# huawei-noah/xingtian

Hardware: NVIDIA H100
Metric: learner env-steps/sec (Atari 84x84x4 PPO) (higher is better)
Workload: dtype f32 (bf16x3 split on wgmma, fp32 accumulate in registers)

## Files before the change

### include/xtb200.h

```cpp
#ifndef XTB200_H_
#define XTB200_H_

#include <stddef.h>
#include <stdint.h>

#ifdef __cplusplus
extern "C" {
#endif

#define XTB_VERSION 101

enum xtb_status {
  XTB_OK = 0,
  XTB_ERR_ARG = -1,
  XTB_ERR_CUDA = -2,
  XTB_ERR_STATE = -3,
  XTB_ERR_NOMEM = -4
};

enum xtb_layer_kind { XTB_CONV = 0, XTB_DENSE = 1, XTB_DUELING = 2, XTB_LOGSTD = 3 };
enum xtb_act {
  XTB_ACT_NONE = 0, XTB_ACT_RELU = 1, XTB_ACT_TANH = 2, XTB_ACT_SIGMOID = 3, XTB_ACT_SOFTSIGN = 4, XTB_ACT_SOFTPLUS = 5,
  XTB_ACT_LEAKY_RELU = 6, XTB_ACT_ELU = 7, XTB_ACT_SELU = 8, XTB_ACT_SWISH = 9, XTB_ACT_GELU = 10
};
// ... 120 lines not shown
  const void* obs;
  const void* action;
  const float* old_logp;
  const float* adv;
  const float* old_v;
  const float* target_v;
} xtb_ppo_rollout;
int xtb_ppo_train(xtb_net* net, xtb_adam* opt, const xtb_ppo_rollout* ro, int n_sample, int batch_size, int n_epoch,
                  const int32_t* perm, const xtb_ppo_hyper* hp, int pi_tensor, int v_tensor, int logstd_tensor,
                  float* loss_per_step, int use_graph, void* stream);

int xtb_impala_train(xtb_net* net, xtb_adam* opt, const void* obs, const int32_t* gather_idx, const float* bp_logits,
                     const int32_t* action, const uint8_t* done, const float* reward, int n_sample, int step_len,
                     float gamma, int logit_tensor, int base_tensor, float* loss_out, int use_graph, void* stream);
int xtb_dqn_train(xtb_net* net, xtb_net* target, xtb_adam* opt, const void* obs, const void* next_obs,
                  const int32_t* idx, const int32_t* action, const float* reward, const uint8_t* done,
                  const float* disc, int n_sample, float gamma, float huber_delta, int q_tensor, float* qn_t,
                  float* qn_o, float* loss_out, int use_graph, void* stream);

int xtb_impala_keras_fit(xtb_net* net, xtb_adam* opt, const void* obs, const int32_t* order, const float* action_mat,
                         const float* adv, const float* target_v, int n, int fit_batch, int logit_tensor, int v_tensor,
                         float ent_coef, float* loss_out, int use_graph, void* stream);
typedef struct xtb_impala_traj {
  const void* obs;
  const float* behav_prob;
  const float* action_mat;
  const float* reward;
  const uint8_t* done;
} xtb_impala_traj;
int xtb_impala_keras_train(xtb_net* net, xtb_adam* opt, const xtb_impala_traj* tr, int n_traj, int ep_len, int slice,
                           int fit_batch, const int32_t* order, int32_t* obs_idx, float gamma, float ent_coef,
                           int logit_tensor, int v_tensor, float* pg_adv, float* target_v, float* loss_per_slice,
                           int use_graph, void* stream);

int xtb_ppo_rollout_infer(xtb_net* net, const void* obs, const int32_t* step_idx, int n_env, int n_step, int pi_tensor,
                          int v_tensor, int logstd_tensor, uint64_t seed, unsigned long long* offset_dev, void* action,
                          float* logp, float* value, int use_graph, void* stream);

int xtb_ppo_predict_host(xtb_net* net, const void* obs_host, size_t obs_bytes, void* obs_dev, int n_env, int pi_tensor,
                         int v_tensor, int logstd_tensor, uint64_t seed, unsigned long long* offset_dev, float* out_dev,
                         float* out_host, float* head_host, int use_graph, void* stream);

int xtb_diag_gaussian_sample(const float* mean, const float* log_std, int batch, int adim, const float* normals,
                             uint64_t seed, uint64_t offset, float* action, float* logp, void* stream);
int xtb_ppo_gauss_loss_grad(const float* mean, const float* v, const float* log_std, const int32_t* gather_idx,
                            const float* action, const float* old_logp, const float* adv, const float* old_v,
                            const float* target_v, int batch, int adim, const xtb_ppo_hyper* hp, float inv_count,
                            float* dmean, float* dv, float* dlog_std, float* loss_out, void* stream);

typedef struct xtb_muzero xtb_muzero;
typedef struct xtb_muzero_desc {
  int32_t unroll;
  int32_t rep_h;
  int32_t dyn_h, dyn_r;
  int32_t pred_p, pred_v;
  float value_min, value_max;
  float reward_min, reward_max;
} xtb_muzero_desc;
int xtb_muzero_create(xtb_net* rep, xtb_net* dyn, xtb_net* pred, const xtb_muzero_desc* desc, int max_batch, xtb_muzero** out);
void xtb_muzero_destroy(xtb_muzero* mz);
typedef struct xtb_muzero_batch {
  const void* obs;
  const int32_t* action;
  const float* target_value;
  const float* target_reward;
  const float* target_policy;
  int32_t unroll;
} xtb_muzero_batch;
int xtb_muzero_train(xtb_muzero* mz, xtb_adam* opt, const xtb_muzero_batch* batch_in, int batch, float loss_offset,
                     float* loss_out, float* value_out, int use_graph, void* stream);
int xtb_muzero_initial_inference(xtb_muzero* mz, const void* obs, int batch, float* hidden_out, float* value_out,
                                 float* policy_out, int use_graph, void* stream);
int xtb_muzero_recurrent_inference(xtb_muzero* mz, const float* hidden, const int32_t* action, int batch, float* hidden_out,
                                   float* reward_out, float* value_out, float* policy_out, int use_graph, void* stream);
typedef struct xtb_muzero_tree xtb_muzero_tree;
int xtb_muzero_tree_create(const xtb_muzero* mz, int max_envs, int max_simulations, xtb_muzero_tree** out);
void xtb_muzero_tree_destroy(xtb_muzero_tree* tree);
int xtb_muzero_search(xtb_muzero* mz, xtb_muzero_tree* tree, const void* obs, int n_envs, int num_simulations,
                      const double* noise, double pb_c_base, double pb_c_init, double discount, double exploration_frac,
                      int32_t* visit_counts_out, double* root_value_out, int use_graph, void* stream);
typedef struct xtb_qmix xtb_qmix;
typedef struct xtb_qmix_desc {
  int32_t batch;
  int32_t episode_limit;
  int32_t n_agents;
  int32_t use_double_q;
  float gamma;
  long long gru_off;
} xtb_qmix_desc;
int xtb_qmix_create(xtb_net* fc1, xtb_net* fc2, xtb_net* hyper, const xtb_qmix_desc* desc, xtb_qmix** out);
void xtb_qmix_destroy(xtb_qmix* q);
typedef struct xtb_qmix_batch {
  const float* obs;
  const int32_t* seq_len;
  const float* avail;
  const int32_t* actions;
  const float* state;
  const float* next_state;
  const float* reward;
  const float* terminated;
  const float* mask;
} xtb_qmix_batch;
int xtb_qmix_train(xtb_qmix* q, xtb_adam* opt, const float* target, const xtb_qmix_batch* batch, float* loss_out, int use_graph,
                   void* stream);
int xtb_qmix_infer(xtb_qmix* q, const float* explore, const float* obs, float* hidden, float* q_out, int use_graph, void* stream);

typedef struct xtb_scc xtb_scc;
#define XTB_SCC_MAX_GROUPS 8
typedef struct xtb_scc_desc {
  int32_t batch;
  int32_t episode_limit;
  int32_t n_agents;
  int32_t n_groups;
  int32_t group[XTB_SCC_MAX_GROUPS];
  int32_t channel_merge;
  int32_t mc_sample_times;
  float gamma;
  long long gru_off;
  long long head_off;
} xtb_scc_desc;
int xtb_scc_create(xtb_net* fc1, xtb_net* fc2, xtb_net* const* critic, const xtb_scc_desc* desc, xtb_scc** out);
void xtb_scc_destroy(xtb_scc* q);
typedef struct xtb_scc_batch {
  const float* obs;
  const float* raw_obs;
  const int32_t* seq_len;
  const int32_t* actions;
  const float* reward;
  const float* terminated;
  const float* mask;
  const uint32_t* subsets;
} xtb_scc_batch;
int xtb_scc_train(xtb_scc* q, xtb_adam* critic_opt, xtb_adam* actor_opt, const float* target, const xtb_scc_batch* batch,
                  float* loss_out, int use_graph, void* stream);
int xtb_scc_infer(xtb_scc* q, const float* explore, const float* obs, float* hidden, float* q_out, int use_graph, void* stream);
int xtb_scc_critic(xtb_scc* q, const float* states, int rows, float* v_out, int use_graph, void* stream);

int xtb_net_backward_input(xtb_net* net, const void* obs, const int32_t* gather_idx, int batch,
                           const int32_t* head_tensors, int n_heads, float* dobs, void* stream);

typedef struct xtb_comm xtb_comm;
int xtb_comm_unique_id(const char* nccl_path, void* id128);
int xtb_comm_create(const char* nccl_path, const void* id128, int rank, int world, xtb_comm** out);
void xtb_comm_destroy(xtb_comm* comm);
int xtb_comm_world(const xtb_comm* comm);
int xtb_set_grad_comm(xtb_comm* comm);
int xtb_comm_allreduce(xtb_comm* comm, float* buf, long long count, void* stream);

int xtb_net_bench_layer(xtb_net* net, int layer, int which, const void* obs, const int32_t* gather_idx,
                        int batch, void* stream);

int xtb_set_tc_mode(int mode);
int xtb_set_fuse_heads(int on);
int xtb_get_tc_mode(void);
int xtb_tc_gemm_test(int mode, const float* a, const float* b, float* c, int M, int N, int K, int ksplit,
                     void* stream);

void* xtb_pinned_alloc(size_t bytes);
void xtb_pinned_free(void* p);
int xtb_copy_h2d(void* dst_dev, const void* src_host, size_t bytes, void* stream);
int xtb_copy_h2d_staged(void* dst_dev, const void* src_host, size_t bytes, void* stream);
int xtb_copy_d2h(void* dst_host, const void* src_dev, size_t bytes, void* stream);
int xtb_stream_sync(void* stream);

#ifdef __cplusplus
}
#endif
#endif
```

### xingtian_b200/capi.py

```python
import ctypes as C
import os

HERE = os.path.dirname(os.path.abspath(__file__))
LIB_PATH = os.environ.get("XTB_LIB_PATH") or os.path.join(HERE, "lib", "libxtb200.so")

XTB_MAX_LAYERS = 16
CONV, DENSE, DUELING, LOGSTD = 0, 1, 2, 3
ACT = {None: 0, "linear": 0, "relu": 1, "tanh": 2, "sigmoid": 3, "softsign": 4, "softplus": 5, "leaky_relu": 6, "elu": 7,
       "selu": 8, "swish": 9, "gelu": 10}
CLIP_NONE, CLIP_GLOBAL_NORM, CLIP_PER_TENSOR = 0, 1, 2


class LayerDesc(C.Structure):
    _fields_ = [("kind", C.c_int32), ("src", C.c_int32), ("act", C.c_int32), ("k", C.c_int32),
                ("stride", C.c_int32), ("cout", C.c_int32), ("pad_same", C.c_int32)]


class NetDesc(C.Structure):
    _fields_ = [("input_u8", C.c_int32), ("scale", C.c_float), ("in_h", C.c_int32), ("in_w", C.c_int32),
                ("in_c", C.c_int32), ("n_layers", C.c_int32), ("layers", LayerDesc * XTB_MAX_LAYERS)]


class LayerPlan(C.Structure):
    _fields_ = [("kind", C.c_int32), ("tc", C.c_int32), ("s2d", C.c_int32), ("w_res", C.c_int32), ("n_fwd", C.c_int32),
                ("n_dg", C.c_int32), ("R", C.c_int32), ("fwd_stages", C.c_int32), ("dg_stages", C.c_int32),
                ("dg_empty_units", C.c_int32), ("k_slices", C.c_int32)]


class PpoHyper(C.Structure):
    _fields_ = [("clip_ratio", C.c_float), ("ent_coef", C.c_float), ("vf_clip", C.c_float),
                ("critic_coef", C.c_float)]


class PpoRollout(C.Structure):
    _fields_ = [("obs", C.c_void_p), ("action", C.c_void_p), ("old_logp", C.c_void_p), ("adv", C.c_void_p),
                ("old_v", C.c_void_p), ("target_v", C.c_void_p)]


class ImpalaTraj(C.Structure):
    _fields_ = [("obs", C.c_void_p), ("behav_prob", C.c_void_p), ("action_mat", C.c_void_p), ("reward", C.c_void_p),
                ("done", C.c_void_p)]


class MuzeroDesc(C.Structure):
    _fields_ = [("unroll", C.c_int32), ("rep_h", C.c_int32), ("dyn_h", C.c_int32), ("dyn_r", C.c_int32), ("pred_p", C.c_int32),
                ("pred_v", C.c_int32), ("value_min", C.c_float), ("value_max", C.c_float), ("reward_min", C.c_float),
                ("reward_max", C.c_float)]


class MuzeroBatch(C.Structure):
    _fields_ = [("obs", C.c_void_p), ("action", C.c_void_p), ("target_value", C.c_void_p), ("target_reward", C.c_void_p),
                ("target_policy", C.c_void_p), ("unroll", C.c_int32)]


class QmixDesc(C.Structure):
    _fields_ = [("batch", C.c_int32), ("episode_limit", C.c_int32), ("n_agents", C.c_int32), ("use_double_q", C.c_int32),
                ("gamma", C.c_float), ("gru_off", C.c_longlong)]


class QmixBatch(C.Structure):
    _fields_ = [("obs", C.c_void_p), ("seq_len", C.c_void_p), ("avail", C.c_void_p), ("actions", C.c_void_p), ("state", C.c_void_p),
                ("next_state", C.c_void_p), ("reward", C.c_void_p), ("terminated", C.c_void_p), ("mask", C.c_void_p)]


class SccDesc(C.Structure):
    _fields_ = [("batch", C.c_int32), ("episode_limit", C.c_int32), ("n_agents", C.c_int32), ("n_groups", C.c_int32),
                ("group", C.c_int32 * 8), ("channel_merge", C.c_int32), ("mc_sample_times", C.c_int32), ("gamma", C.c_float),
                ("gru_off", C.c_longlong), ("head_off", C.c_longlong)]


class SccBatch(C.Structure):
    _fields_ = [("obs", C.c_void_p), ("raw_obs", C.c_void_p), ("seq_len", C.c_void_p), ("actions", C.c_void_p), ("reward", C.c_void_p),
                ("terminated", C.c_void_p), ("mask", C.c_void_p), ("subsets", C.c_void_p)]


_P = C.c_void_p
_SIGS = {
    "xtb_version": (C.c_int, []),
    "xtb_last_error": (C.c_char_p, []),
    "xtb_launch_count": (C.c_longlong, []),
    "xtb_graph_replay_count": (C.c_longlong, []),
    "xtb_net_create": (C.c_int, [C.POINTER(NetDesc), C.c_int, C.POINTER(_P)]),
    "xtb_net_destroy": (None, [_P]),
    "xtb_net_param_count": (C.c_longlong, [_P]),
    "xtb_net_layer_params": (C.c_int, [_P, C.c_int, C.POINTER(C.c_longlong), C.POINTER(C.c_longlong),
                                       C.POINTER(C.c_int), C.POINTER(C.c_int)]),
    "xtb_net_layer_plan": (C.c_int, [_P, C.c_int, C.POINTER(LayerPlan)]),
    "xtb_net_tensor_size": (C.c_int, [_P, C.c_int]),
    "xtb_net_workspace_bytes": (C.c_size_t, [_P]),
    "xtb_net_bind": (C.c_int, [_P, _P, _P, _P, C.c_size_t]),
    "xtb_net_bind_stream": (C.c_int, [_P, _P, _P, _P, C.c_size_t, _P]),
    "xtb_net_sync_weights": (C.c_int, [_P, _P]),
    "xtb_net_tensor": (_P, [_P, C.c_int]),
    "xtb_net_tensor_grad": (_P, [_P, C.c_int]),
    "xtb_net_forward": (C.c_int, [_P, _P, _P, _P, C.c_int, _P]),
    "xtb_net_backward": (C.c_int, [_P, _P, _P, C.c_int, C.POINTER(C.c_int32), C.c_int, _P]),
    "xtb_categorical_sample": (C.c_int, [_P, C.c_int, C.c_int, _P, C.c_uint64, C.c_uint64, _P, _P, _P]),
    "xtb_argmax": (C.c_int, [_P, C.c_int, C.c_int, _P, _P]),
    "xtb_gae": (C.c_int, [_P, _P, _P, C.c_int, C.c_int, C.c_float, C.c_float, C.c_int, _P, _P, _P, _P]),
    "xtb_ppo_loss_grad": (C.c_int, [_P, _P, _P, _P, _P, _P, _P, _P, C.c_int, C.c_int, C.POINTER(PpoHyper),
                                    C.c_float, _P, _P, _P, _P]),
    "xtb_vtrace_loss_grad": (C.c_int, [_P, _P, _P, _P, _P, _P, C.c_int, C.c_int, C.c_int, C.c_float,
                                       _P, _P, _P, _P, _P, _P]),
    "xtb_dqn_loss_grad": (C.c_int, [_P, _P, _P, _P, _P, _P, C.c_int, C.c_int, C.c_float, C.c_float,
                                    _P, _P, _P, _P]),
    "xtb_dqn_td_loss_grad": (C.c_int, [_P, _P, _P, _P, _P, _P, _P, _P, C.c_int, C.c_int, C.c_float, C.c_float, C.c_float,
                                      _P, _P, _P, _P]),
    "xtb_nstep_returns": (C.c_int, [_P, _P, C.c_int, C.c_int, C.c_int, C.c_float, _P, _P, _P, _P, _P]),
    "xtb_impala_train": (C.c_int, [_P, _P, _P, _P, _P, _P, _P, _P, C.c_int, C.c_int, C.c_float, C.c_int, C.c_int, _P, C.c_int, _P]),
    "xtb_dqn_train": (C.c_int, [_P, _P, _P, _P, _P, _P, _P, _P, _P, _P, C.c_int, C.c_float, C.c_float, C.c_int, _P, _P, _P,
                               C.c_int, _P]),
    "xtb_mse_loss_grad": (C.c_int, [_P, _P, C.c_int, C.c_int, C.c_float, _P, _P, _P]),
    "xtb_softmax": (C.c_int, [_P, C.c_int, C.c_int, _P, _P]),
    "xtb_impala_keras_loss_grad": (C.c_int, [_P, _P, _P, _P, _P, _P, C.c_int, C.c_int, C.c_float, C.c_float, C.c_float,
                                             _P, _P, _P, _P]),
    "xtb_impala_keras_fit": (C.c_int, [_P, _P, _P, _P, _P, _P, _P, C.c_int, C.c_int, C.c_int, C.c_int, C.c_float, _P,
                                       C.c_int, _P]),
    "xtb_impala_keras_train": (C.c_int, [_P, _P, C.POINTER(ImpalaTraj), C.c_int, C.c_int, C.c_int, C.c_int, _P, _P,
                                         C.c_float, C.c_float, C.c_int, C.c_int, _P, _P, _P, C.c_int, _P]),
    "xtb_adam_create": (C.c_int, [C.c_longlong, C.c_float, C.c_float, C.c_float, C.c_float, C.c_int,
                                  C.c_float, C.POINTER(C.c_longlong), C.c_int, _P, _P, C.POINTER(_P)]),
    "xtb_adam_destroy": (None, [_P]),
    "xtb_adam_step": (C.c_int, [_P, _P, _P, C.c_float, _P]),
    "xtb_adam_step_net": (C.c_int, [_P, _P, C.c_float, _P]),
    "xtb_adam_grad_norm": (_P, [_P]),
    "xtb_adam_set_lr": (C.c_int, [_P, C.c_float]),
    "xtb_adam_set_decay": (C.c_int, [_P, C.c_float]),
    "xtb_opt_use_rmsprop": (C.c_int, [_P, _P, C.c_float, C.c_float]),
    "xtb_opt_use_rmsprop_plain": (C.c_int, [_P, C.c_float, C.c_float]),
    "xtb_ppo_train": (C.c_int, [_P, _P, C.POINTER(PpoRollout), C.c_int, C.c_int, C.c_int, _P, C.POINTER(PpoHyper),
                                C.c_int, C.c_int, C.c_int, _P, C.c_int, _P]),
    "xtb_ppo_rollout_infer": (C.c_int, [_P, _P, _P, C.c_int, C.c_int, C.c_int, C.c_int, C.c_int, C.c_uint64, _P, _P, _P, _P,
                                        C.c_int, _P]),
    "xtb_ppo_predict_host": (C.c_int, [_P, _P, C.c_size_t, _P, C.c_int, C.c_int, C.c_int, C.c_int, C.c_uint64, _P, _P, _P, _P,
                                       C.c_int, _P]),
    "xtb_ppo_heads_plan": (C.c_int, [_P, C.c_int, C.c_int, C.c_int, C.POINTER(C.c_int), C.POINTER(C.c_int)]),
    "xtb_diag_gaussian_sample": (C.c_int, [_P, _P, C.c_int, C.c_int, _P, C.c_uint64, C.c_uint64, _P, _P, _P]),
    "xtb_ppo_gauss_loss_grad": (C.c_int, [_P, _P, _P, _P, _P, _P, _P, _P, _P, C.c_int, C.c_int, C.POINTER(PpoHyper), C.c_float,
                                          _P, _P, _P, _P, _P]),
    "xtb_muzero_create": (C.c_int, [_P, _P, _P, C.POINTER(MuzeroDesc), C.c_int, C.POINTER(_P)]),
    "xtb_muzero_destroy": (None, [_P]),
    "xtb_muzero_train": (C.c_int, [_P, _P, C.POINTER(MuzeroBatch), C.c_int, C.c_float, _P, _P, C.c_int, _P]),
    "xtb_muzero_initial_inference": (C.c_int, [_P, _P, C.c_int, _P, _P, _P, C.c_int, _P]),
    "xtb_muzero_recurrent_inference": (C.c_int, [_P, _P, _P, C.c_int, _P, _P, _P, _P, C.c_int, _P]),
    "xtb_muzero_tree_create": (C.c_int, [_P, C.c_int, C.c_int, C.POINTER(_P)]),
    "xtb_muzero_tree_destroy": (None, [_P]),
    "xtb_muzero_search": (C.c_int, [_P, _P, _P, C.c_int, C.c_int, _P, C.c_double, C.c_double, C.c_double, C.c_double, _P, _P,
                                    C.c_int, _P]),
    "xtb_qmix_create": (C.c_int, [_P, _P, _P, C.POINTER(QmixDesc), C.POINTER(_P)]),
    "xtb_qmix_destroy": (None, [_P]),
    "xtb_qmix_train": (C.c_int, [_P, _P, _P, C.POINTER(QmixBatch), _P, C.c_int, _P]),
    "xtb_qmix_infer": (C.c_int, [_P, _P, _P, _P, _P, C.c_int, _P]),
    "xtb_scc_create": (C.c_int, [_P, _P, C.POINTER(_P), C.POINTER(SccDesc), C.POINTER(_P)]),
    "xtb_scc_destroy": (None, [_P]),
    "xtb_scc_train": (C.c_int, [_P, _P, _P, _P, C.POINTER(SccBatch), _P, C.c_int, _P]),
    "xtb_scc_infer": (C.c_int, [_P, _P, _P, _P, _P, C.c_int, _P]),
    "xtb_scc_critic": (C.c_int, [_P, _P, C.c_int, _P, C.c_int, _P]),
    "xtb_net_backward_input": (C.c_int, [_P, _P, _P, C.c_int, C.POINTER(C.c_int32), C.c_int, _P, _P]),
    "xtb_comm_unique_id": (C.c_int, [C.c_char_p, _P]),
    "xtb_comm_create": (C.c_int, [C.c_char_p, _P, C.c_int, C.c_int, C.POINTER(_P)]),
    "xtb_comm_destroy": (None, [_P]),
    "xtb_comm_world": (C.c_int, [_P]),
    "xtb_set_grad_comm": (C.c_int, [_P]),
    "xtb_comm_allreduce": (C.c_int, [_P, _P, C.c_longlong, _P]),
    "xtb_net_bench_layer": (C.c_int, [_P, C.c_int, C.c_int, _P, _P, C.c_int, _P]),
    "xtb_set_fuse_heads": (C.c_int, [C.c_int]),
    "xtb_set_tc_mode": (C.c_int, [C.c_int]),
    "xtb_get_tc_mode": (C.c_int, []),
    "xtb_tc_gemm_test": (C.c_int, [C.c_int, _P, _P, _P, C.c_int, C.c_int, C.c_int, C.c_int, _P]),
    "xtb_pinned_alloc": (_P, [C.c_size_t]),
    "xtb_pinned_free": (None, [_P]),
    "xtb_copy_h2d": (C.c_int, [_P, _P, C.c_size_t, _P]),
    "xtb_copy_h2d_staged": (C.c_int, [_P, _P, C.c_size_t, _P]),
    "xtb_copy_d2h": (C.c_int, [_P, _P, C.c_size_t, _P]),
    "xtb_stream_sync": (C.c_int, [_P]),
}

EXPORTED = tuple(_SIGS)
_lib = None


def lib():
    global _lib
    if _lib is None:
        if not os.path.exists(LIB_PATH):
            raise RuntimeError(
                "xingtian_b200: CUDA library %s is missing -- run `python -m xingtian_b200.build` "
                "(there is no CPU fallback)" % LIB_PATH)
        handle = C.CDLL(LIB_PATH)
        for name, (res, args) in _SIGS.items():
            fn = getattr(handle, name)
            fn.restype = res
            fn.argtypes = args
        _lib = handle
    return _lib


def check(rc):
    if rc != 0:
        raise RuntimeError("xtb200 error %d: %s" % (rc, lib().xtb_last_error().decode()))
```

### xingtian_b200/csrc/bp_gemm.cuh

```cuda
#pragma once
#include <cuda_bf16.h>
#include <cuda_runtime.h>
#include <stdint.h>

#include "gemm_f32.cuh"

#ifndef XTB_BP_WAIT_HINT
#define XTB_BP_WAIT_HINT 20000u
#endif

namespace xtb {
namespace bp {

typedef __nv_bfloat16 bf16;

__device__ __forceinline__ uint32_t smem_u32(const void* p) { return (uint32_t)__cvta_generic_to_shared(p); }
__device__ __forceinline__ void mbar_init(uint32_t bar, uint32_t count) {
  asm volatile("mbarrier.init.shared::cta.b64 [%0], %1;" ::"r"(bar), "r"(count) : "memory");
}
__device__ __forceinline__ void fence_barrier_init() { asm volatile("fence.mbarrier_init.release.cluster;" ::: "memory"); }
__device__ __forceinline__ void mbar_arrive(uint32_t bar) {
  asm volatile("mbarrier.arrive.shared::cta.b64 _, [%0];" ::"r"(bar) : "memory");
}
__device__ __forceinline__ void mbar_expect_tx(uint32_t bar, uint32_t bytes) {
// ... 70 lines not shown
      "wgmma.mma_async.sync.aligned.m64n32k16.f32.bf16.bf16 {%0, %1, %2, %3, %4, %5, %6, %7, %8, %9, %10, %11, %12, %13, %14, %15}, %16, %17, p, 1, 1, %19, %20;\n\t}"
      : "+f"(d[0]), "+f"(d[1]), "+f"(d[2]), "+f"(d[3]),
        "+f"(d[4]), "+f"(d[5]), "+f"(d[6]), "+f"(d[7]),
        "+f"(d[8]), "+f"(d[9]), "+f"(d[10]), "+f"(d[11]),
        "+f"(d[12]), "+f"(d[13]), "+f"(d[14]), "+f"(d[15])
      : "l"(a), "l"(b), "r"(scale_d), "n"(TA), "n"(TB));
}
template <int TA, int TB>
__device__ __forceinline__ void wgmma_n48(float* d, uint64_t a, uint64_t b, uint32_t scale_d) {
  asm volatile(
      "{\n\t.reg .pred p;\n\tsetp.ne.b32 p, %26, 0;\n\t"
      "wgmma.mma_async.sync.aligned.m64n48k16.f32.bf16.bf16 {%0, %1, %2, %3, %4, %5, %6, %7, %8, %9, %10, %11, %12, %13, %14, %15, %16, %17, %18, %19, %20, %21, %22, %23}, %24, %25, p, 1, 1, %27, %28;\n\t}"
      : "+f"(d[0]), "+f"(d[1]), "+f"(d[2]), "+f"(d[3]),
        "+f"(d[4]), "+f"(d[5]), "+f"(d[6]), "+f"(d[7]),
        "+f"(d[8]), "+f"(d[9]), "+f"(d[10]), "+f"(d[11]),
        "+f"(d[12]), "+f"(d[13]), "+f"(d[14]), "+f"(d[15]),
        "+f"(d[16]), "+f"(d[17]), "+f"(d[18]), "+f"(d[19]),
        "+f"(d[20]), "+f"(d[21]), "+f"(d[22]), "+f"(d[23])
      : "l"(a), "l"(b), "r"(scale_d), "n"(TA), "n"(TB));
}
template <int TA, int TB>
__device__ __forceinline__ void wgmma_n64(float* d, uint64_t a, uint64_t b, uint32_t scale_d) {
  asm volatile(
      "{\n\t.reg .pred p;\n\tsetp.ne.b32 p, %34, 0;\n\t"
      "wgmma.mma_async.sync.aligned.m64n64k16.f32.bf16.bf16 {%0, %1, %2, %3, %4, %5, %6, %7, %8, %9, %10, %11, %12, %13, %14, %15, %16, %17, %18, %19, %20, %21, %22, %23, %24, %25, %26, %27, %28, %29, %30, %31}, %32, %33, p, 1, 1, %35, %36;\n\t}"
      : "+f"(d[0]), "+f"(d[1]), "+f"(d[2]), "+f"(d[3]),
        "+f"(d[4]), "+f"(d[5]), "+f"(d[6]), "+f"(d[7]),
        "+f"(d[8]), "+f"(d[9]), "+f"(d[10]), "+f"(d[11]),
        "+f"(d[12]), "+f"(d[13]), "+f"(d[14]), "+f"(d[15]),
        "+f"(d[16]), "+f"(d[17]), "+f"(d[18]), "+f"(d[19]),
        "+f"(d[20]), "+f"(d[21]), "+f"(d[22]), "+f"(d[23]),
        "+f"(d[24]), "+f"(d[25]), "+f"(d[26]), "+f"(d[27]),
        "+f"(d[28]), "+f"(d[29]), "+f"(d[30]), "+f"(d[31])
      : "l"(a), "l"(b), "r"(scale_d), "n"(TA), "n"(TB));
}
template <int TA, int TB>
__device__ __forceinline__ void wgmma_n96(float* d, uint64_t a, uint64_t b, uint32_t scale_d) {
  asm volatile(
      "{\n\t.reg .pred p;\n\tsetp.ne.b32 p, %50, 0;\n\t"
      "wgmma.mma_async.sync.aligned.m64n96k16.f32.bf16.bf16 {%0, %1, %2, %3, %4, %5, %6, %7, %8, %9, %10, %11, %12, %13, %14, %15, %16, %17, %18, %19, %20, %21, %22, %23, %24, %25, %26, %27, %28, %29, %30, %31, %32, %33, %34, %35, %36, %37, %38, %39, %40, %41, %42, %43, %44, %45, %46, %47}, %48, %49, p, 1, 1, %51, %52;\n\t}"
      : "+f"(d[0]), "+f"(d[1]), "+f"(d[2]), "+f"(d[3]),
        "+f"(d[4]), "+f"(d[5]), "+f"(d[6]), "+f"(d[7]),
        "+f"(d[8]), "+f"(d[9]), "+f"(d[10]), "+f"(d[11]),
        "+f"(d[12]), "+f"(d[13]), "+f"(d[14]), "+f"(d[15]),
        "+f"(d[16]), "+f"(d[17]), "+f"(d[18]), "+f"(d[19]),
        "+f"(d[20]), "+f"(d[21]), "+f"(d[22]), "+f"(d[23]),
        "+f"(d[24]), "+f"(d[25]), "+f"(d[26]), "+f"(d[27]),
        "+f"(d[28]), "+f"(d[29]), "+f"(d[30]), "+f"(d[31]),
        "+f"(d[32]), "+f"(d[33]), "+f"(d[34]), "+f"(d[35]),
        "+f"(d[36]), "+f"(d[37]), "+f"(d[38]), "+f"(d[39]),
        "+f"(d[40]), "+f"(d[41]), "+f"(d[42]), "+f"(d[43]),
        "+f"(d[44]), "+f"(d[45]), "+f"(d[46]), "+f"(d[47])
      : "l"(a), "l"(b), "r"(scale_d), "n"(TA), "n"(TB));
}
template <int TA, int TB>
__device__ __forceinline__ void wgmma_n128(float* d, uint64_t a, uint64_t b, uint32_t scale_d) {
  asm volatile(
      "{\n\t.reg .pred p;\n\tsetp.ne.b32 p, %66, 0;\n\t"
      "wgmma.mma_async.sync.aligned.m64n128k16.f32.bf16.bf16 {%0, %1, %2, %3, %4, %5, %6, %7, %8, %9, %10, %11, %12, %13, %14, %15, %16, %17, %18, %19, %20, %21, %22, %23, %24, %25, %26, %27, %28, %29, %30, %31, %32, %33, %34, %35, %36, %37, %38, %39, %40, %41, %42, %43, %44, %45, %46, %47, %48, %49, %50, %51, %52, %53, %54, %55, %56, %57, %58, %59, %60, %61, %62, %63}, %64, %65, p, 1, 1, %67, %68;\n\t}"
      : "+f"(d[0]), "+f"(d[1]), "+f"(d[2]), "+f"(d[3]),
        "+f"(d[4]), "+f"(d[5]), "+f"(d[6]), "+f"(d[7]),
        "+f"(d[8]), "+f"(d[9]), "+f"(d[10]), "+f"(d[11]),
        "+f"(d[12]), "+f"(d[13]), "+f"(d[14]), "+f"(d[15]),
        "+f"(d[16]), "+f"(d[17]), "+f"(d[18]), "+f"(d[19]),
        "+f"(d[20]), "+f"(d[21]), "+f"(d[22]), "+f"(d[23]),
        "+f"(d[24]), "+f"(d[25]), "+f"(d[26]), "+f"(d[27]),
        "+f"(d[28]), "+f"(d[29]), "+f"(d[30]), "+f"(d[31]),
        "+f"(d[32]), "+f"(d[33]), "+f"(d[34]), "+f"(d[35]),
        "+f"(d[36]), "+f"(d[37]), "+f"(d[38]), "+f"(d[39]),
        "+f"(d[40]), "+f"(d[41]), "+f"(d[42]), "+f"(d[43]),
        "+f"(d[44]), "+f"(d[45]), "+f"(d[46]), "+f"(d[47]),
        "+f"(d[48]), "+f"(d[49]), "+f"(d[50]), "+f"(d[51]),
        "+f"(d[52]), "+f"(d[53]), "+f"(d[54]), "+f"(d[55]),
        "+f"(d[56]), "+f"(d[57]), "+f"(d[58]), "+f"(d[59]),
        "+f"(d[60]), "+f"(d[61]), "+f"(d[62]), "+f"(d[63])
      : "l"(a), "l"(b), "r"(scale_d), "n"(TA), "n"(TB));
}
template <int N, int TA, int TB>
__device__ __forceinline__ void wgmma(float* d, uint64_t a, uint64_t b, uint32_t scale_d = 1) {
  static_assert(N == 16 || N == 32 || N == 48 || N == 64 || N == 96 || N == 128, "wgmma width");
  if constexpr (N == 16) wgmma_n16<TA, TB>(d, a, b, scale_d);
  else if constexpr (N == 32) wgmma_n32<TA, TB>(d, a, b, scale_d);
  else if constexpr (N == 48) wgmma_n48<TA, TB>(d, a, b, scale_d);
  else if constexpr (N == 64) wgmma_n64<TA, TB>(d, a, b, scale_d);
  else if constexpr (N == 96) wgmma_n96<TA, TB>(d, a, b, scale_d);
  else wgmma_n128<TA, TB>(d, a, b, scale_d);
}

__device__ __forceinline__ uint32_t pack_bf16(float a, float b) {
  __nv_bfloat162 t = __floats2bfloat162_rn(a, b);
  return *reinterpret_cast<uint32_t*>(&t);
}
__device__ __forceinline__ void split2(float a, float b, uint32_t& hi, uint32_t& lo) {
  hi = pack_bf16(a, b);
  float ha = __uint_as_float(hi << 16), hb = __uint_as_float(hi & 0xffff0000u);
  lo = pack_bf16(a - ha, b - hb);
}
__device__ __forceinline__ void unpack2(uint32_t w, float& a, float& b) {
  a = __uint_as_float(w << 16);
  b = __uint_as_float(w & 0xffff0000u);
}
__device__ __forceinline__ void unpack8(const uint4& u, float v[8]) {
  const uint32_t w[4] = {u.x, u.y, u.z, u.w};
#pragma unroll
  for (int i = 0; i < 4; i++) unpack2(w[i], v[2 * i], v[2 * i + 1]);
}
__device__ __forceinline__ void split8(const float v[8], uint4& hi, uint4& lo) {
  split2(v[0], v[1], hi.x, lo.x);
  split2(v[2], v[3], hi.y, lo.y);
  split2(v[4], v[5], hi.z, lo.z);
  split2(v[6], v[7], hi.w, lo.w);
}

struct BpT {
  bf16* hi;
  long long lo_off;
  int pitch;
};
__host__ __device__ inline long long bp_index(int pitch, int row, int f) { return ((long long)(f >> 3) * pitch + row) * 8 + (f & 7); }

constexpr int BP_CONSUMER_WGS = 2;
constexpr int BP_P_WARP = 4 * BP_CONSUMER_WGS;
constexpr int BP_THREADS = 32 * (BP_P_WARP + 1);
constexpr int BP_CONSUMER_WARPS = 4 * BP_CONSUMER_WGS;

constexpr int RW_THREADS = BP_THREADS;
constexpr int RW_A_PLANE = 2048;
constexpr int RW_STAGE_A = 2 * 8 * RW_A_PLANE;
constexpr int RW_STAGE_B = 16384;
constexpr int RW_MAX_STAGES = 4;
constexpr int RW_EPI_BANKS = 2;

__host__ __device__ inline int dgrad_epi_planes(int src_act, int accumulate) {
  return (src_act == 1 ? 1 : (src_act == 2 ? 2 : 0)) + (accumulate ? 2 : 0);
}

struct StageEnt {
  uint32_t a_chunk;
  uint16_t w_row;
  uint16_t nch;
};
typedef uint32_t UnitEnt;
struct StageDesc { uint32_t a_off, w_off, nch; };

struct RowsArgs {
  BpT a; int a_split;
  const bf16* w_hi; const bf16* w_lo; int w_pitch;
  int w_res; int w_res_chunks;
  int mode;
  const StageEnt* stages; const UnitEnt* units;
  int n_stage_ents;
  int kchunks, kc_split, n_ntiles;
  int n_units, n_btiles, B, N;
  BpT out; float* out_f32; int ld_f32; const float* bias; float alpha; int act;
  float* part; long long part_z; int ld_part;
  BpT src; int src_act; int accumulate; float* db_part;
};

struct TileWalk {
  const uint2* stages_sm; const uint32_t* units_sm;
  uint32_t a_pstride, w_pitch; int mode, n_ntiles, kc_split, kchunks, N;
  const uint2* st; uint32_t a0, w0, da, dw; int ns, nch_last;
  __device__ __forceinline__ void setup(const RowsArgs& a, const uint2* s_sm, const uint32_t* u_sm) {
    stages_sm = s_sm; units_sm = u_sm;
    a_pstride = (uint32_t)a.a.pitch * 16u; w_pitch = (uint32_t)a.w_pitch;
    mode = a.mode; n_ntiles = a.n_ntiles; kc_split = a.kc_split; kchunks = a.kchunks; N = a.N;
  }
  template <int KIND>
  __device__ __forceinline__ void init(int u) {
    if (mode == 2) {
      const int nt = u % n_ntiles, z = u / n_ntiles;
      const int cbeg = z * kc_split, cend = min(kchunks, cbeg + kc_split);
      ns = (cend - cbeg + 7) >> 3;
      nch_last = cend - cbeg - 8 * (ns - 1);
      a0 = (uint32_t)cbeg * a_pstride; da = 8u * a_pstride;
      if (KIND == 2) { w0 = ((uint32_t)cbeg * w_pitch + (uint32_t)nt * N) * 16u; dw = 8u * w_pitch * 16u; }
      else { w0 = ((uint32_t)(nt * (N >> 3)) * w_pitch + (uint32_t)cbeg * 8u) * 16u; dw = 1024u; }
      st = nullptr;
    } else {
      const uint32_t ue = units_sm[u];
      st = stages_sm + (ue & 0xffffffu); ns = (int)(ue >> 24);
    }
  }
  __device__ __forceinline__ StageDesc get(int s) const {
    if (st) {
      const uint2 v = st[s];
      return StageDesc{v.x * a_pstride, (v.y & 0xffffu) * 16u, v.y >> 16};
    }
    return StageDesc{a0 + (uint32_t)s * da, w0 + (uint32_t)s * dw, (uint32_t)(s == ns - 1 ? nch_last : 8)};
  }
};

template <int KIND, int N>
__global__ void __launch_bounds__(RW_THREADS, 1)
bp_rows_kernel(const __grid_constant__ RowsArgs a, int n_stages, int stage_bytes, int wres_bytes, int epi_banks) {
  extern __shared__ uint8_t smem_raw[];
  uint8_t* smem = reinterpret_cast<uint8_t*>((reinterpret_cast<uintptr_t>(smem_raw) + 127) & ~(uintptr_t)127);
  constexpr int NCH = N >> 3;
  const int epi_planes = KIND == 2 ? dgrad_epi_planes(a.src_act, a.accumulate) : 0;
  const int epi_bank_bytes = epi_planes * NCH * RW_A_PLANE;
  uint8_t* epi_sm = smem + wres_bytes + n_stages * stage_bytes;
  uint2* stages_sm = reinterpret_cast<uint2*>(epi_sm + epi_banks * epi_bank_bytes);
  uint32_t* units_sm = reinterpret_cast<uint32_t*>(stages_sm + a.n_stage_ents);
  __shared__ __align__(8) uint64_t bars[2 * RW_MAX_STAGES + 1 + 2 * RW_EPI_BANKS];
  __shared__ float red_sh[BP_CONSUMER_WARPS][64];
  __shared__ float bias_sh[64];

  const int tid = threadIdx.x, warp = __shfl_sync(0xffffffffu, tid >> 5, 0), lane = tid & 31;
  const uint32_t full0 = smem_u32(&bars[0]), empty0 = smem_u32(&bars[RW_MAX_STAGES]), wbar = smem_u32(&bars[2 * RW_MAX_STAGES]);
  const uint32_t efull0 = wbar + 8, eempty0 = efull0 + 8 * RW_EPI_BANKS;
  if (tid == 0) {
    for (int s = 0; s < RW_MAX_STAGES; s++) { mbar_init(full0 + 8 * s, 1); mbar_init(empty0 + 8 * s, BP_CONSUMER_WARPS); }
    mbar_init(wbar, 1);
    for (int k = 0; k < RW_EPI_BANKS; k++) { mbar_init(efull0 + 8 * k, 1); mbar_init(eempty0 + 8 * k, BP_CONSUMER_WARPS); }
    fence_barrier_init();
  }
  __syncthreads();
  if (a.mode != 2) {
    const uint2* gs = reinterpret_cast<const uint2*>(a.stages);
    for (int i = tid; i < a.n_stage_ents; i += RW_THREADS) stages_sm[i] = __ldg(gs + i);
    for (int i = tid; i < a.n_units; i += RW_THREADS) units_sm[i] = __ldg(a.units + i);
  }
  if (warp == BP_P_WARP && a.w_res && elect_one()) {
    const uint32_t bytes = (uint32_t)a.w_res_chunks * a.w_pitch * 16;
    mbar_expect_tx(wbar, 2 * bytes);
    bulk_g2s(smem_u32(smem), a.w_hi, bytes, wbar);
    bulk_g2s(smem_u32(smem) + bytes, a.w_lo, bytes, wbar);
  }
  pdl_wait();
  pdl_trigger();
  if (KIND == 0 && a.mode != 2 && tid < N) bias_sh[tid] = a.bias[tid];
  __syncthreads();
  const uint32_t wres = smem_u32(smem);
  const uint32_t stage0 = wres + (uint32_t)wres_bytes;
  const int total = a.n_units * a.n_btiles;
  constexpr bool CAT = (KIND != 2);
  const int nbt = a.n_btiles;
  const int du = (int)gridDim.x / nbt, dbt = (int)gridDim.x - du * nbt;

  if (warp == BP_P_WARP) {
    const bool a_split = a.a_split != 0, w_res = a.w_res != 0;
    const uint32_t a_pstride = (uint32_t)a.a.pitch * 16u, w_pstride = (uint32_t)a.w_pitch * 16u;
    const char* a_hi = reinterpret_cast<const char*>(a.a.hi);
    const char* a_lo = a_hi + a.a.lo_off * 2;
    const char* w_hi = reinterpret_cast<const char*>(a.w_hi);
    const char* w_lo = reinterpret_cast<const char*>(a.w_lo);
    constexpr int n_bh_fwd = N >> 3;
    int stage = 0; uint32_t phase = 0;
    int u = (int)blockIdx.x / nbt, bt = (int)blockIdx.x - u * nbt;
    const int Bsz = a.B;
    TileWalk tw; tw.setup(a, stages_sm, units_sm);
    const int src_act = a.src_act, accumulate = a.accumulate;
    const char* s_hi = reinterpret_cast<const char*>(a.src.hi);
    const char* s_lo = s_hi + a.src.lo_off * 2;
    const char* o_hi = reinterpret_cast<const char*>(a.out.hi);
    const char* o_lo = o_hi + a.out.lo_off * 2;
    const uint32_t s_ps = (uint32_t)a.src.pitch * 16u, o_ps = (uint32_t)a.out.pitch * 16u;
    int ebank = 0; uint32_t ephase = 0;
    for (int tile = blockIdx.x; tile < total; tile += gridDim.x) {
      const int b0 = bt * 128, nr = min(128, Bsz - b0);
      const uint32_t a_bytes = (uint32_t)nr * 16u, row_off = (uint32_t)b0 * 16u;
      tw.init<KIND>(u);
      for (int s = 0; s < tw.ns; s++) {
        const StageDesc d = tw.get(s);
        mbar_wait(empty0 + 8 * stage, phase ^ 1);
        const int nch = (int)d.nch;
        const int n_bh = w_res ? 0 : (KIND == 2 ? nch : n_bh_fwd);
        const uint32_t b_bytes = (KIND == 2) ? (uint32_t)N * 16u : (uint32_t)nch * 128u;
        const uint32_t fb = full0 + 8 * stage;
        if (elect_one()) {
          mbar_expect_tx(fb, a_bytes * (a_split ? 2 * nch : nch) + b_bytes * 2 * n_bh);
          const uint32_t sA = stage0 + (uint32_t)stage * stage_bytes, sB = sA + RW_STAGE_A;
          const char* ah = a_hi + d.a_off + row_off;
          for (int c = 0; c < nch; c++) bulk_g2s(sA + c * RW_A_PLANE, ah + (uint32_t)c * a_pstride, a_bytes, fb);
          if (a_split) {
            const char* al = a_lo + d.a_off + row_off;
            for (int c = 0; c < nch; c++) bulk_g2s(sA + 8 * RW_A_PLANE + c * RW_A_PLANE, al + (uint32_t)c * a_pstride, a_bytes, fb);
          }
          if (!w_res) {
            const char* wh = w_hi + d.w_off; const char* wl = w_lo + d.w_off;
            if (KIND == 2) {
              for (int c = 0; c < n_bh; c++) {
                bulk_g2s(sB + c * (N * 16), wh + (uint32_t)c * w_pstride, b_bytes, fb);
                bulk_g2s(sB + 8192 + c * (N * 16), wl + (uint32_t)c * w_pstride, b_bytes, fb);
              }
            } else {
              for (int c = 0; c < n_bh; c++) {
                bulk_g2s(sB + c * 1024, wh + (uint32_t)c * w_pstride, b_bytes, fb);
                bulk_g2s(sB + (n_bh_fwd + c) * 1024, wl + (uint32_t)c * w_pstride, b_bytes, fb);
              }
            }
          }
        }
        __syncwarp();
        if (++stage == n_stages) { stage = 0; phase ^= 1; }
      }
      if (KIND == 2 && epi_planes) {
        mbar_wait(eempty0 + 8 * ebank, ephase ^ 1);
        if (elect_one()) {
          const uint32_t fb = efull0 + 8 * ebank;
          mbar_expect_tx(fb, a_bytes * (uint32_t)(NCH * epi_planes));
          const uint32_t oc0 = (uint32_t)((tw.mode == 2 ? u % tw.n_ntiles : u) * NCH);
          uint32_t dst = smem_u32(epi_sm) + (uint32_t)(ebank * epi_bank_bytes);
          auto plane = [&](const char* base, uint32_t ps) {
            const char* src = base + oc0 * ps + row_off;
            for (int c = 0; c < NCH; c++, dst += RW_A_PLANE) bulk_g2s(dst, src + (uint32_t)c * ps, a_bytes, fb);
          };
          if (src_act == 1 || src_act == 2) plane(s_hi, s_ps);
          if (src_act == 2) plane(s_lo, s_ps);
          if (accumulate) { plane(o_hi, o_ps); plane(o_lo, o_ps); }
        }
        __syncwarp();
        if (++ebank == epi_banks) { ebank = 0; ephase ^= 1; }
      }
      u += du; bt += dbt;
      if (bt >= nbt) { bt -= nbt; u++; }
    }
  } else if (warp < BP_P_WARP) {
    constexpr int ACC = CAT ? 2 * N : N;
    float dbacc[N / 4];
#pragma unroll
    for (int j = 0; j < N / 4; j++) dbacc[j] = 0.f;
    const int wg = warp >> 2, q = lane & 3;
    const int row_in_tile = wg * 64 + (warp & 3) * 16 + (lane >> 2);
    const bool a_split = a.a_split != 0, w_res = a.w_res != 0;
    const int act = a.act, mode = a.mode, Bsz = a.B, n_nt = a.n_ntiles, ld_f32 = a.ld_f32, src_act = a.src_act, accumulate = a.accumulate;
    const int ld_part = a.ld_part;
    const float alpha = a.alpha;
    bf16* const out_hi = a.out.hi; const long long out_lo = a.out.lo_off;
    float* const out_f32 = a.out_f32; const float* const bias_g = a.bias;
    float* const part = a.part; const long long part_z = a.part_z;
    const long long out_pstride = (long long)a.out.pitch * 8;
    const int b_pad = (Bsz + 15) & ~15;
    const uint32_t epi_thr = smem_u32(epi_sm) + (uint32_t)(row_in_tile * 16 + 4 * q);
    const int epi_out_plane = epi_planes - (accumulate ? 2 : 0);
    int ebank = 0; uint32_t ephase = 0;
    const uint64_t adesc = make_desc(0, RW_A_PLANE, 128);
    const uint64_t bdesc = (KIND == 2) ? make_desc(0, (uint32_t)N * 16, 128) : make_desc(0, 128, 1024);
    const uint32_t a_row_add = (uint32_t)(wg * 64 * 16) >> 4;
    const uint32_t a_lo_add = (8 * RW_A_PLANE) >> 4, a_step = (2 * RW_A_PLANE) >> 4;
    const uint32_t w_pstride = (uint32_t)a.w_pitch * 16u;
    const uint64_t wdesc = (KIND == 2) ? make_desc(0, w_pstride, 128) : make_desc(0, 128, w_pstride);
    const uint32_t w_lo_add = ((uint32_t)a.w_res_chunks * w_pstride) >> 4;
    const uint32_t b_step = (KIND == 2) ? (w_res ? (2 * w_pstride) >> 4 : (2u * N * 16u) >> 4) : (256 >> 4);
    const uint32_t b_lo_add = w_res ? w_lo_add : (8192 >> 4);
    const uint64_t b_const = w_res ? wdesc : bdesc;
    if (w_res) mbar_wait(wbar, 0);
    int stage = 0; uint32_t phase = 0;
    int held = -1;
    auto idle = [&](int bt) { return bt * 128 + wg * 64 >= Bsz; };

    auto mma_stage = [&](float* acc, const StageDesc& d, bool first, bool skip) {
      mbar_wait(full0 + 8 * stage, phase);
      const uint32_t sA = stage0 + (uint32_t)stage * stage_bytes;
      uint32_t a_lo32 = (sA >> 4) + a_row_add;
      uint32_t b_lo32 = w_res ? (wres + d.w_off) >> 4 : (sA + RW_STAGE_A) >> 4;
      const int ksteps = __shfl_sync(0xffffffffu, skip ? 0 : (int)d.nch >> 1, 0);
      uint32_t sd = first ? 0u : 1u;
      wgmma_fence();
      if (a_split) {
        for (int j = 0; j < ksteps; j++) {
          const uint64_t ah = adesc | a_lo32, bh = b_const | b_lo32, al = adesc | (a_lo32 + a_lo_add);
          if (KIND != 2) {
            wgmma<2 * N, 0, 1>(acc, ah, bh, sd);
            wgmma<N, 0, 1>(acc, al, bh);
          } else {
            wgmma<N, 0, 0>(acc, ah, bh, sd);
            wgmma<N, 0, 0>(acc, ah, b_const | (b_lo32 + b_lo_add));
            wgmma<N, 0, 0>(acc, al, bh);
          }
          a_lo32 += a_step; b_lo32 += b_step; sd = 1u;
        }
      } else {
        for (int j = 0; j < ksteps; j++) {
          const uint64_t ah = adesc | a_lo32, bh = b_const | b_lo32;
          if (KIND != 2) {
            wgmma<2 * N, 0, 1>(acc, ah, bh, sd);
          } else {
            wgmma<N, 0, 0>(acc, ah, bh, sd);
            wgmma<N, 0, 0>(acc, ah, b_const | (b_lo32 + b_lo_add));
          }
          a_lo32 += a_step; b_lo32 += b_step; sd = 1u;
        }
      }
      wgmma_commit();
      wgmma_wait<1>();
      if (held >= 0 && lane == 0) mbar_arrive(empty0 + 8 * held);
      held = stage;
      if (++stage == n_stages) { stage = 0; phase ^= 1; }
    };

    int tile = blockIdx.x;
    int u = (int)blockIdx.x / nbt, bt = (int)blockIdx.x - u * nbt;
    TileWalk tw; tw.setup(a, stages_sm, units_sm);
    auto start_tile = [&](float* acc) {
      tw.init<KIND>(u);
      tw.ns = __shfl_sync(0xffffffffu, tw.ns, 0);
      if (tw.ns == 0) return false;
      discard_regs<ACC / 2>(acc);
      mma_stage(acc, tw.get(0), true, idle(bt));
      return true;
    };

    auto epilogue = [&](const float* cur, int cu, int cbt, bool empty, uint32_t eb) {
      const int btile0 = cbt * 128;
      int oc0, z = 0;
      if (mode == 2) { const int nt = cu % n_nt; z = cu / n_nt; oc0 = nt * NCH; }
      else oc0 = cu * NCH;
#pragma unroll
      for (int h = 0; h < 2; h++) {
        const int b = btile0 + row_in_tile + 8 * h;
#pragma unroll
        for (int i = 0; i < NCH; i++) {
          const int c = 8 * i + 2 * q;
          float v0 = cur[4 * i + 2 * h], v1 = cur[4 * i + 2 * h + 1];
          if (CAT) { v0 += cur[4 * (i + NCH) + 2 * h]; v1 += cur[4 * (i + NCH) + 2 * h + 1]; }
          if (empty) { v0 = 0.f; v1 = 0.f; }
          if (KIND == 0) {
            if (b < Bsz) {
              const int f = oc0 * 8 + c;
              float bb0, bb1;
              if (mode == 2) { const float2 t2 = __ldg(reinterpret_cast<const float2*>(bias_g + f)); bb0 = t2.x; bb1 = t2.y; }
              else { bb0 = bias_sh[c]; bb1 = bias_sh[c + 1]; }
              if (act == 2) { v0 = tanhf(alpha * v0 + bb0); v1 = tanhf(alpha * v1 + bb1); }
              else {
                const float lo = act == 1 ? 0.f : -INFINITY;
                v0 = fmaxf(fmaf(alpha, v0, bb0), lo); v1 = fmaxf(fmaf(alpha, v1, bb1), lo);
              }
              if (out_hi) {
                bf16* p = out_hi + (long long)(oc0 + i) * out_pstride + (long long)b * 8 + 2 * q;
                uint32_t hi, lo;
                split2(v0, v1, hi, lo);
                *reinterpret_cast<uint32_t*>(p) = hi;
                *reinterpret_cast<uint32_t*>(p + out_lo) = lo;
              }
              if (out_f32) *reinterpret_cast<float2*>(out_f32 + (long long)b * ld_f32 + f) = make_float2(v0, v1);
            }
          } else if (KIND == 1) {
            if (b < Bsz)
              *reinterpret_cast<float2*>(part + (long long)z * part_z + (long long)b * ld_part + oc0 * 8 + c) = make_float2(v0, v1);
          } else {
            bf16* p = out_hi + (long long)(oc0 + i) * out_pstride + (long long)b * 8 + 2 * q;
            if (b < Bsz) {
              const uint32_t e = eb + (uint32_t)(i * RW_A_PLANE + 128 * h);
              if (src_act == 1) {
                float s0, s1;
                unpack2(lds_u32(e), s0, s1);
                v0 = s0 > 0.f ? v0 : 0.f; v1 = s1 > 0.f ? v1 : 0.f;
              } else if (src_act == 2) {
                float s0, s1, t0, t1;
                unpack2(lds_u32(e), s0, s1);
                unpack2(lds_u32(e + NCH * RW_A_PLANE), t0, t1);
                const float y0 = s0 + t0, y1 = s1 + t1;
                v0 *= 1.f - y0 * y0; v1 *= 1.f - y1 * y1;
              }
              dbacc[2 * i] += v0; dbacc[2 * i + 1] += v1;
              if (accumulate) {
                const uint32_t eo = e + (uint32_t)(epi_out_plane * NCH * RW_A_PLANE);
                float s0, s1, t0, t1;
                unpack2(lds_u32(eo), s0, s1);
                unpack2(lds_u32(eo + NCH * RW_A_PLANE), t0, t1);
                v0 += s0 + t0; v1 += s1 + t1;
              }
              uint32_t hi, lo;
              split2(v0, v1, hi, lo);
              *reinterpret_cast<uint32_t*>(p) = hi;
              *reinterpret_cast<uint32_t*>(p + out_lo) = lo;
            } else if (b < b_pad && !accumulate) {
              *reinterpret_cast<uint32_t*>(p) = 0u;
              *reinterpret_cast<uint32_t*>(p + out_lo) = 0u;
            }
          }
        }
      }
    };

    constexpr bool OVERLAP = !(KIND == 0 && N == 64);
    auto finish_tile = [&](float* cur, float* nxt) {
      for (int s = 1; s < tw.ns; s++) mma_stage(cur, tw.get(s), false, idle(bt));
      const bool empty = tw.ns == 0;
      const int cu = u, cbt = bt;
      tile += gridDim.x; u += du; bt += dbt;
      if (bt >= nbt) { bt -= nbt; u++; }
      if (!(OVERLAP && tile < total && start_tile(nxt))) {
        wgmma_wait<0>();
        if (held >= 0 && lane == 0) mbar_arrive(empty0 + 8 * held);
        held = -1;
      }
      fence_regs<ACC / 2>(cur);
      if (KIND == 2 && epi_planes) mbar_wait(efull0 + 8 * ebank, ephase);
      if (!idle(cbt)) epilogue(cur, cu, cbt, empty, epi_thr + (uint32_t)(ebank * epi_bank_bytes));
      if (KIND == 2 && epi_planes) {
        __syncwarp();
        if (lane == 0) mbar_arrive(eempty0 + 8 * ebank);
        if (++ebank == epi_banks) { ebank = 0; ephase ^= 1; }
      }
      if (!OVERLAP && tile < total) start_tile(nxt);
    };
    float acc0[ACC / 2], acc1[ACC / 2];
    if (tile < total) start_tile(acc0);
    while (tile < total) {
      finish_tile(acc0, acc1);
      if (tile >= total) break;
      finish_tile(acc1, acc0);
    }
    if (KIND == 2 && a.db_part) {
#pragma unroll
      for (int j = 0; j < N / 4; j++) {
        float s = dbacc[j];
        s += __shfl_xor_sync(0xffffffffu, s, 4);
        s += __shfl_xor_sync(0xffffffffu, s, 8);
        s += __shfl_xor_sync(0xffffffffu, s, 16);
        if (lane < 4) red_sh[warp][8 * (j >> 1) + 2 * lane + (j & 1)] = s;
      }
      asm volatile("bar.sync 1, %0;" ::"n"(32 * BP_CONSUMER_WARPS) : "memory");
      if (tid < N) {
        float t = 0.f;
#pragma unroll
        for (int w = 0; w < BP_CONSUMER_WARPS; w++) t += red_sh[w][tid];
        a.db_part[(long long)blockIdx.x * N + tid] = t;
      }
    }
  }
}

constexpr int WG_KB = 64;
constexpr int WG_PLANE = WG_KB * 16;
constexpr int WG_STAGE_A = 2 * 16 * WG_PLANE;
constexpr int WG_STAGE_B = 2 * 8 * WG_PLANE;
constexpr int WG_STAGE = WG_STAGE_A + WG_STAGE_B;
constexpr int WG_STAGES = 4;
constexpr int WG_THREADS = BP_THREADS;

struct WgEnt {
  int32_t x_chunk;
  uint16_t okmask;
  uint16_t valid;
};

struct WgradArgs {
  BpT x; int x_split; BpT g; const bf16* zeros;
  int mode;
  const WgEnt* tab;
  int R;
  int N, B, n_bsub, n_opix;
  int x_chunks, r_tiles, n_ntiles;
  float* part;
  float* dw; int ldw; int k_rows;
};

struct WgWalk {
  __device__ __forceinline__ static WgEnt get(const WgradArgs& a, const uint2* tab_sm, int opix, int r, int rt) {
    if (a.mode == 0) {
      const uint2 v = tab_sm[opix * a.R + r];
      return WgEnt{(int32_t)v.x, (uint16_t)(v.y & 0xffffu), (uint16_t)(v.y >> 16)};
    }
    const int c0 = rt * 16, left = a.x_chunks - c0;
    return WgEnt{c0, (uint16_t)(left >= 16 ? 0xffffu : ((1u << left) - 1u)), (uint16_t)1};
  }
};

template <int N>
__global__ void __launch_bounds__(WG_THREADS, 1)
bp_wgrad_kernel(const __grid_constant__ WgradArgs a) {
  extern __shared__ uint8_t smem_raw[];
  uint8_t* smem = reinterpret_cast<uint8_t*>((reinterpret_cast<uintptr_t>(smem_raw) + 127) & ~(uintptr_t)127);
  __shared__ __align__(8) uint64_t bars[2 * WG_STAGES];
  uint2* tab_sm = reinterpret_cast<uint2*>(smem + WG_STAGES * WG_STAGE);

  const int tid = threadIdx.x, warp = __shfl_sync(0xffffffffu, tid >> 5, 0), lane = tid & 31;
  const uint32_t full0 = smem_u32(&bars[0]), empty0 = smem_u32(&bars[WG_STAGES]);
  if (tid == 0) {
    for (int s = 0; s < WG_STAGES; s++) { mbar_init(full0 + 8 * s, 1); mbar_init(empty0 + 8 * s, BP_CONSUMER_WARPS); }
    fence_barrier_init();
  }
  const bool conv = a.mode == 0;
  if (conv) {
    const uint2* gt = reinterpret_cast<const uint2*>(a.tab);
    for (int i = tid; i < a.n_opix * a.R; i += WG_THREADS) tab_sm[i] = __ldg(gt + i);
  }
  __syncthreads();
  pdl_wait();
  pdl_trigger();
  const uint32_t stage0 = smem_u32(smem);
  const int n_slices = conv ? (int)gridDim.x / a.R : 1;
  const int r_conv = conv ? (int)blockIdx.x / n_slices : 0, slice = conv ? (int)blockIdx.x - r_conv * n_slices : 0;
  const int n_tiles = conv ? 1 : a.r_tiles * a.n_ntiles;
  const int n_kc = conv ? a.n_opix * a.n_bsub : a.n_bsub;
  const int tile0 = conv ? 0 : (int)blockIdx.x, tile_step = conv ? 1 : (int)gridDim.x;
  const int kc0 = conv ? slice : 0, kc_step = conv ? n_slices : 1;

  if (warp == BP_P_WARP) {
    const uint32_t pstride_x = (uint32_t)a.x.pitch * 16u, pstride_g = (uint32_t)a.g.pitch * 16u;
    const char* x_hi = reinterpret_cast<const char*>(a.x.hi);
    const char* x_lo = x_hi + a.x.lo_off * 2;
    const char* g_hi = reinterpret_cast<const char*>(a.g.hi);
    const char* g_lo = g_hi + a.g.lo_off * 2;
    const char* zeros = reinterpret_cast<const char*>(a.zeros);
    const bool x_split = a.x_split != 0;
    constexpr int n_bh = N >> 3;
    int stage = 0; uint32_t phase = 0;
    for (int tile = tile0; tile < n_tiles; tile += tile_step) {
      const int rt = tile / a.n_ntiles, nt = tile - rt * a.n_ntiles;
      for (int kc = kc0; kc < n_kc; kc += kc_step) {
        const int opix = conv ? kc / a.n_bsub : 0, bs = conv ? kc - opix * a.n_bsub : kc;
        const WgEnt e = WgWalk::get(a, tab_sm, opix, r_conv, rt);
        if (!e.valid) continue;
        const int b0 = bs * WG_KB;
        const uint32_t bytes = (uint32_t)((min(WG_KB, a.B - b0) + 15) & ~15) * 16u, row_off = (uint32_t)b0 * 16u;
        const uint32_t g_off = (uint32_t)((conv ? opix : nt) * n_bh) * pstride_g + row_off;
        const long long x_off = (long long)e.x_chunk * (long long)pstride_x + row_off;
        mbar_wait(empty0 + 8 * stage, phase ^ 1);
        const uint32_t fb = full0 + 8 * stage;
        if (elect_one()) {
          mbar_expect_tx(fb, bytes * ((x_split ? 32 : 16) + 2 * n_bh));
          const uint32_t sA = stage0 + (uint32_t)stage * WG_STAGE, sB = sA + WG_STAGE_A;
          const uint32_t mask = e.okmask;
#pragma unroll 4
          for (int c = 0; c < 16; c++)
            bulk_g2s(sA + c * WG_PLANE, ((mask >> c) & 1u) ? x_hi + x_off + (long long)((uint32_t)c * pstride_x) : zeros, bytes, fb);
          if (x_split) {
#pragma unroll 4
            for (int c = 0; c < 16; c++)
              bulk_g2s(sA + (16 + c) * WG_PLANE, ((mask >> c) & 1u) ? x_lo + x_off + (long long)((uint32_t)c * pstride_x) : zeros, bytes, fb);
          }
          for (int c = 0; c < n_bh; c++) {
            bulk_g2s(sB + c * WG_PLANE, g_hi + g_off + (uint32_t)c * pstride_g, bytes, fb);
            bulk_g2s(sB + (8 + c) * WG_PLANE, g_lo + g_off + (uint32_t)c * pstride_g, bytes, fb);
          }
        }
        __syncwarp();
        if (++stage == WG_STAGES) { stage = 0; phase ^= 1; }
      }
    }
  } else if (warp < BP_P_WARP) {
    float acc[N / 2];
    const int wg = warp >> 2, q = lane & 3;
    const bool x_split = a.x_split != 0;
    const uint64_t desc = make_desc(0, 128, WG_PLANE);
    const uint32_t x_row_add = (uint32_t)(wg * 8 * WG_PLANE) >> 4;
    int stage = 0; uint32_t phase = 0;
    for (int tile = tile0; tile < n_tiles; tile += tile_step) {
      const int rt = tile / a.n_ntiles, nt = tile - rt * a.n_ntiles;
#pragma unroll
      for (int j = 0; j < N / 2; j++) acc[j] = 0.f;
      int held = -1;
      for (int kc = kc0; kc < n_kc; kc += kc_step) {
        const int opix = conv ? kc / a.n_bsub : 0, bs = conv ? kc - opix * a.n_bsub : kc;
        if (!__shfl_sync(0xffffffffu, (int)WgWalk::get(a, tab_sm, opix, r_conv, rt).valid, 0)) continue;
        const int ksteps = __shfl_sync(0xffffffffu, ((min(WG_KB, a.B - bs * WG_KB) + 15) & ~15) >> 4, 0);
        mbar_wait(full0 + 8 * stage, phase);
        const uint32_t sA = stage0 + (uint32_t)stage * WG_STAGE;
        uint32_t x32 = (sA >> 4) + x_row_add, g32 = (sA + WG_STAGE_A) >> 4;
        wgmma_fence();
        if (x_split) {
          for (int j = 0; j < ksteps; j++) {
            const uint64_t xh = desc | x32, gh = desc | g32;
            wgmma<N, 1, 1>(acc, xh, gh);
            wgmma<N, 1, 1>(acc, xh, desc | (g32 + ((8 * WG_PLANE) >> 4)));
            wgmma<N, 1, 1>(acc, desc | (x32 + ((16 * WG_PLANE) >> 4)), gh);
            x32 += 256 >> 4; g32 += 256 >> 4;
          }
        } else {
          for (int j = 0; j < ksteps; j++) {
            const uint64_t xh = desc | x32;
            wgmma<N, 1, 1>(acc, xh, desc | g32);
            wgmma<N, 1, 1>(acc, xh, desc | (g32 + ((8 * WG_PLANE) >> 4)));
            x32 += 256 >> 4; g32 += 256 >> 4;
          }
        }
        wgmma_commit();
        wgmma_wait<1>();
        if (held >= 0 && lane == 0) mbar_arrive(empty0 + 8 * held);
        held = stage;
        if (++stage == WG_STAGES) { stage = 0; phase ^= 1; }
      }
      wgmma_wait<0>();
      fence_regs<N / 2>(acc);
      if (held >= 0 && lane == 0) mbar_arrive(empty0 + 8 * held);
#pragma unroll
      for (int h = 0; h < 2; h++) {
        const int m = wg * 64 + (warp & 3) * 16 + (lane >> 2) + 8 * h;
        float* dst;
        bool ok;
        if (conv) {
          dst = a.part + (((long long)slice * a.R + r_conv) * 128 + m) * N;
          ok = true;
        } else {
          const int k = rt * 128 + m;
          dst = a.dw + (long long)k * a.ldw + nt * N;
          ok = k < a.k_rows;
        }
        if (ok) {
#pragma unroll
          for (int i = 0; i < N / 8; i++)
            *reinterpret_cast<float2*>(dst + 8 * i + 2 * q) = make_float2(acc[4 * i + 2 * h], acc[4 * i + 2 * h + 1]);
        }
      }
    }
  }
}

struct RedSeg {
  const float* part; int n_slabs; long long slab;
  int count;
  int kind;
  int N, C, KW, mts, s2d_k4;
  long long dst_off; float alpha;
  float* dst_ptr;
};
__host__ __device__ inline int s2d_real_row(int m, int k4) {
  int tap = m >> 6, ty = tap / k4, tx = tap - ty * k4;
  int dy = (m >> 4) & 3, dx = (m >> 2) & 3, c = m & 3;
  return (((4 * ty + dy) * 4 * k4 + 4 * tx + dx) << 2) + c;
}
constexpr int RED_MAX = 24;
struct RedSegs { RedSeg s[RED_MAX]; };
__global__ void __launch_bounds__(256) grad_reduce_kernel(const __grid_constant__ RedSegs segs, float* __restrict__ grads) {
  pdl_wait(); pdl_trigger();
  __shared__ float4 sh[8][32];
  const RedSeg& s = segs.s[blockIdx.y];
  if ((int)blockIdx.x * 128 >= s.count) return;
  const int lane = threadIdx.x & 31, w = threadIdx.x >> 5;
  const int i = ((int)blockIdx.x * 32 + lane) * 4;
  float4 acc = make_float4(0.f, 0.f, 0.f, 0.f);
  if (i < s.count) {
    const bool vec = ((s.count | (int)(s.slab & 3)) & 3) == 0 && (reinterpret_cast<unsigned long long>(s.part) & 15ull) == 0;
    if (vec) {
#pragma unroll 5
      for (int k = w; k < s.n_slabs; k += 8) {
        const float4 x = *reinterpret_cast<const float4*>(s.part + (long long)k * s.slab + i);
        acc.x += x.x; acc.y += x.y; acc.z += x.z; acc.w += x.w;
      }
    } else {
      for (int k = w; k < s.n_slabs; k += 8) {
        const float* p = s.part + (long long)k * s.slab + i;
        acc.x += p[0];
        if (i + 1 < s.count) acc.y += p[1];
        if (i + 2 < s.count) acc.z += p[2];
        if (i + 3 < s.count) acc.w += p[3];
      }
    }
  }
  sh[w][lane] = acc;
  __syncthreads();
  if (w != 0 || i >= s.count) return;
  float4 t = sh[0][lane];
#pragma unroll
  for (int q = 1; q < 8; q++) { const float4 x = sh[q][lane]; t.x += x.x; t.y += x.y; t.z += x.z; t.w += x.w; }
  const float v[4] = {t.x, t.y, t.z, t.w};
#pragma unroll
  for (int e = 0; e < 4; e++) {
    const int ie = i + e;
    if (ie >= s.count) break;
    long long dst;
    if (s.kind == 0) {
      const int n = ie % s.N, mm = (ie / s.N) & 127, r = ie / (s.N * 128);
      const int ky = r / s.mts, mt = r - ky * s.mts;
      const int feat = mt * 128 + mm;
      if (feat >= s.KW * s.C) continue;
      int row = ky * s.KW * s.C + feat;
      if (s.s2d_k4) row = s2d_real_row(row, s.s2d_k4);
      dst = s.dst_off + (long long)row * s.N + n;
    } else dst = s.dst_off + ie;
    (s.dst_ptr ? s.dst_ptr : grads)[dst] = s.alpha * v[e];
  }
}

__global__ void bp_split_kernel(const float* __restrict__ src, int B, int F, BpT dst) {
  pdl_wait(); pdl_trigger();
  const int b_pad = (B + 15) & ~15;
  const long long i = (long long)blockIdx.x * blockDim.x + threadIdx.x;
  const int chunks = F >> 3;
  if (i >= (long long)chunks * b_pad) return;
  const int c = (int)(i / b_pad), b = (int)(i - (long long)c * b_pad);
  uint4 hi = make_uint4(0, 0, 0, 0), lo = hi;
  if (b < B) {
    const float4* p = reinterpret_cast<const float4*>(src + (long long)b * F + c * 8);
    float4 x = p[0], y = p[1];
    float v[8] = {x.x, x.y, x.z, x.w, y.x, y.y, y.z, y.w};
    split8(v, hi, lo);
  }
  bf16* o = dst.hi + ((long long)c * dst.pitch + b) * 8;
  *reinterpret_cast<uint4*>(o) = hi;
  *reinterpret_cast<uint4*>(o + dst.lo_off) = lo;
}
__global__ void bp_merge_kernel(BpT src, int B, int F, float* __restrict__ dst) {
  pdl_wait(); pdl_trigger();
  const long long i = (long long)blockIdx.x * blockDim.x + threadIdx.x;
  const int chunks = F >> 3;
  if (i >= (long long)chunks * B) return;
  const int c = (int)(i / B), b = (int)(i - (long long)c * B);
  const bf16* p = src.hi + ((long long)c * src.pitch + b) * 8;
  float h[8], l[8];
  unpack8(*reinterpret_cast<const uint4*>(p), h);
  unpack8(*reinterpret_cast<const uint4*>(p + src.lo_off), l);
  float4* o = reinterpret_cast<float4*>(dst + (long long)b * F + c * 8);
  o[0] = make_float4(h[0] + l[0], h[1] + l[1], h[2] + l[2], h[3] + l[3]);
  o[1] = make_float4(h[4] + l[4], h[5] + l[5], h[6] + l[6], h[7] + l[7]);
}
__global__ void bp_colsum_kernel(BpT g, int B, int F, int period, float* __restrict__ db) {
  pdl_wait(); pdl_trigger();
  const int c = blockIdx.x * (blockDim.x >> 5) + (threadIdx.x >> 5), lane = threadIdx.x & 31;
  if (c >= (F >> 3)) return;
  float s[8] = {0, 0, 0, 0, 0, 0, 0, 0};
  for (int b = lane; b < B; b += 32) {
    const bf16* p = g.hi + ((long long)c * g.pitch + b) * 8;
    float h[8], l[8];
    unpack8(*reinterpret_cast<const uint4*>(p), h);
    unpack8(*reinterpret_cast<const uint4*>(p + g.lo_off), l);
#pragma unroll
    for (int i = 0; i < 8; i++) s[i] += h[i] + l[i];
  }
#pragma unroll
  for (int i = 0; i < 8; i++) {
    float v = s[i];
#pragma unroll
    for (int o = 16; o > 0; o >>= 1) v += __shfl_xor_sync(0xffffffffu, v, o);
    if (lane == 0) atomicAdd(db + (c * 8 + i) % period, v);
  }
}
constexpr int FIN_ZL = 8;
__global__ void bp_splitk_finish_kernel(const float* __restrict__ part, int n_z, long long part_z, int B, int N,
                                        const float* __restrict__ bias, int act, float* __restrict__ out_f32, BpT out) {
  pdl_wait(); pdl_trigger();
  const int b_pad = (B + 15) & ~15;
  const long long t = (long long)blockIdx.x * blockDim.x + threadIdx.x;
  const long long i = t / FIN_ZL;
  const int zl = (int)(t - i * FIN_ZL);
  const int chunks = N >> 3;
  const int c = (int)(i / b_pad), b = (int)(i - (long long)c * b_pad);
  const bool valid = i < (long long)chunks * b_pad && b < B;
  float v[8] = {0, 0, 0, 0, 0, 0, 0, 0};
  if (valid) {
    const float* p0 = part + (long long)b * N + c * 8;
#pragma unroll 4
    for (int z = zl; z < n_z; z += FIN_ZL) {
      const float4* p = reinterpret_cast<const float4*>(p0 + (long long)z * part_z);
      float4 x = p[0], y = p[1];
// ... 134 lines not shown
```

### xingtian_b200/csrc/xtb_engine.cu

```cuda
#include "../../include/xtb200.h"

#include <cuda_runtime.h>

#include <atomic>
#include <cmath>
#include <cstdarg>
#include <cstdio>
#include <cstring>
#include <map>
#include <string>
#include <tuple>
#include <vector>

#include "gemm_f32.cuh"
#include "optim.cuh"
#include "rl_kernels.cuh"
#include "qmix.cuh"
#include "scc.cuh"
#include "stager.cuh"
#include "bp_gemm.cuh"
#include "comm.cuh"
#include <cstdlib>
#include <type_traits>

// ... 535 lines not shown
  if (n_cols) *n_cols = lp.N;
  return XTB_OK;
}

extern "C" int xtb_net_layer_plan(const xtb_net* net, int layer, xtb_layer_plan* out) {
  if (!net || !out || layer < 0 || layer >= (int)net->L.size()) return fail(XTB_ERR_ARG, "xtb_net_layer_plan: bad argument");
  const LayerPlan& lp = net->L[layer];
  memset(out, 0, sizeof *out);
  out->kind = lp.d.kind;
  if (!lp.tc) return XTB_OK;
  out->tc = 1; out->s2d = lp.s2d; out->w_res = lp.w_res;
  out->n_fwd = lp.n_fwd; out->n_dg = lp.n_dg; out->R = lp.R;
  if (lp.d.kind == XTB_CONV) {
    out->fwd_stages = rows_smem(lp.w_res, lp.N / 8, lp.K, 0, lp.fwd_st.size(), lp.fwd_un.size(), lp.n_fwd, 0).n_stages;
    out->dg_stages = conv_dgrad_smem(lp, false).n_stages;
    for (bp::UnitEnt u : lp.dg_un) out->dg_empty_units += (u >> 24) == 0;
    out->k_slices = 1;
  } else {
    out->fwd_stages = rows_smem(false, 0, lp.K, 2, 0, 0, lp.n_fwd, 0).n_stages;
    out->dg_stages = rows_smem(false, 0, lp.K, 2, 0, 0, lp.n_dg, bp::dgrad_epi_planes(dgrad_act(lp), 0)).n_stages;
    int kc_split;
    out->k_slices = dense_k_slices(lp.K / 8, (lp.N / lp.n_fwd) * ((net->max_batch + 127) / 128), &kc_split);
  }
  return XTB_OK;
}

extern "C" int xtb_net_tensor_size(const xtb_net* net, int t) {
  if (!net || t < 0 || t >= (int)net->tsize.size()) return -1;
  return net->tsize[t];
}

extern "C" size_t xtb_net_workspace_bytes(const xtb_net* net) { return net ? net->ws_bytes : 0; }

static cudaError_t ensure_kernel_attrs();
extern "C" int xtb_net_sync_weights(xtb_net* net, void* stream);
extern "C" int xtb_net_bind_stream(xtb_net* net, float* params, float* grads, void* workspace, size_t workspace_bytes, void* stream) {
  if (!net || !params || !workspace) return fail(XTB_ERR_ARG, "xtb_net_bind: null pointer");
  if (workspace_bytes < net->ws_bytes) return fail(XTB_ERR_ARG, "workspace too small: %zu < %zu", workspace_bytes, net->ws_bytes);
  bool tc_layers = false;
  for (const auto& lp : net->L) tc_layers |= lp.tc;
  if (tc_layers && (uintptr_t)params % 16) return fail(XTB_ERR_ARG, "xtb_net_bind: parameters must be 16-byte aligned");
  drop_graphs_of(net);
  net->params = params; net->grads = grads; net->ws = (char*)workspace;
  cudaStream_t st = S(stream);
  { cudaError_t ea = ensure_kernel_attrs(); if (ea != cudaSuccess) return fail(XTB_ERR_CUDA, "kernel attributes: %s", cudaGetErrorString(ea)); }
  CUDA_TRY(cudaMemsetAsync(net->ws, 0, net->ws_bytes, st));
  if (!net->blob_segs.empty())
    CUDA_TRY(cudaMemcpyAsync(net->ws + net->segs_off, net->blob_segs.data(), net->blob_segs.size() * sizeof(bp::BlobSeg),
                             cudaMemcpyHostToDevice, st));
  for (const auto& lp : net->L) if (lp.tc && lp.d.kind == XTB_CONV) {
    auto up = [&](size_t off, const void* src, size_t bytes) { return bytes ? cudaMemcpyAsync(net->ws + off, src, bytes, cudaMemcpyHostToDevice, st) : cudaSuccess; };
    CUDA_TRY(up(lp.fwd_st_off, lp.fwd_st.data(), lp.fwd_st.size() * sizeof(bp::StageEnt)));
    CUDA_TRY(up(lp.fwd_un_off, lp.fwd_un.data(), lp.fwd_un.size() * sizeof(bp::UnitEnt)));
    CUDA_TRY(up(lp.dg_st_off, lp.dg_st.data(), lp.dg_st.size() * sizeof(bp::StageEnt)));
    CUDA_TRY(up(lp.dg_un_off, lp.dg_un.data(), lp.dg_un.size() * sizeof(bp::UnitEnt)));
    CUDA_TRY(up(lp.wg_off, lp.wg_tab.data(), lp.wg_tab.size() * sizeof(bp::WgEnt)));
  }
  invalidate(net, true, true);
  int rc = xtb_net_sync_weights(net, stream);
  if (rc) return rc;
  CUDA_TRY(cudaStreamSynchronize(st));
  return XTB_OK;
}
extern "C" int xtb_net_bind(xtb_net* net, float* params, float* grads, void* workspace, size_t workspace_bytes) {
  return xtb_net_bind_stream(net, params, grads, workspace, workspace_bytes, nullptr);
}

extern "C" float* xtb_net_tensor(xtb_net* net, int t) {
  if (!net || !net->ws || t < 1 || t >= (int)net->tsize.size()) return nullptr;
  return out_f32(net, t);
}
extern "C" float* xtb_net_tensor_grad(xtb_net* net, int t) {
  if (!net || !net->ws || t < 1 || t >= (int)net->tsize.size()) return nullptr;
  return gout_f32(net, t);
}

template <int BM, int BN, int TM, int TN, class AL, class BL, class EP>
static void launch_cfg(const AL& al, const BL& bl, const EP& ep, int M, int N, int K, int ksplit, cudaStream_t st) {
  constexpr int BK = 16;
  int kc = (K + ksplit - 1) / ksplit;
  kc = (kc + BK - 1) / BK * BK;
  int ks = (K + kc - 1) / kc;
  dim3 grid((M + BM - 1) / BM, (N + BN - 1) / BN, ks);
  XLAUNCH((gemm_f32_kernel<BM, BN, BK, TM, TN, AL, BL, EP>), grid, (BM / TM) * (BN / TN), 0, st, al, bl, ep, M, N, K, kc);
}

template <class AL, class BL, class EP>
static void launch_gemm(const AL& al, const BL& bl, const EP& ep, int M, int N, int K, bool split_ok, cudaStream_t st) {
  auto ctas = [&](int bm, int bn) { return (long long)((M + bm - 1) / bm) * ((N + bn - 1) / bn); };
  int ksplit = 1;
  if (N <= 32) {
    long long c = ctas(128, 32);
    if (c >= kSMs || split_ok) {
      if (split_ok) { ksplit = (int)((2 * kSMs + c - 1) / c); int mx = (K + 63) / 64; if (ksplit > mx) ksplit = mx; if (ksplit < 1) ksplit = 1; }
      launch_cfg<128, 32, 4, 4>(al, bl, ep, M, N, K, ksplit, st);
      return;
    }
    launch_cfg<32, 32, 2, 2>(al, bl, ep, M, N, K, 1, st);
    return;
  }
  long long c = ctas(64, 64);
  if (c >= kSMs || split_ok) {
    if (split_ok) { ksplit = (int)((2 * kSMs + c - 1) / c); int mx = (K + 63) / 64; if (ksplit > mx) ksplit = mx; if (ksplit < 1) ksplit = 1; }
    launch_cfg<64, 64, 4, 4>(al, bl, ep, M, N, K, ksplit, st);
    return;
  }
  launch_cfg<32, 32, 2, 2>(al, bl, ep, M, N, K, 1, st);
}

template <int KIND>
static void (*const kRowsKernels[])(bp::RowsArgs, int, int, int, int) = {
    bp::bp_rows_kernel<KIND, 16>, bp::bp_rows_kernel<KIND, 32>, bp::bp_rows_kernel<KIND, 48>, bp::bp_rows_kernel<KIND, 64>};
static void (*const kWgradKernels[])(bp::WgradArgs) = {bp::bp_wgrad_kernel<16>, bp::bp_wgrad_kernel<32>,
                                                       bp::bp_wgrad_kernel<48>, bp::bp_wgrad_kernel<64>};
template <class F, size_t C>
static F by_width(F const (&tab)[C], int n) { return n > 0 && n % 16 == 0 && n / 16 <= (int)C ? tab[n / 16 - 1] : nullptr; }

template <class F> struct HeadsEnt { int kpl, amax; F kern; };
template <class LOSS>
static const HeadsEnt<void (*)(PpoHeadsArgs)> kHeadsKernels[] = {
    {2, 8, heads_kernel<LOSS, 2, 8>}, {8, 4, heads_kernel<LOSS, 8, 4>}, {8, 8, heads_kernel<LOSS, 8, 8>},
    {16, 4, heads_kernel<LOSS, 16, 4>}};
template <class DIST>
static const HeadsEnt<decltype(&infer_heads_kernel<DIST, 2, 8>)> kInferHeadsKernels[] = {
    {2, 8, infer_heads_kernel<DIST, 2, 8>}, {8, 4, infer_heads_kernel<DIST, 8, 4>}, {8, 8, infer_heads_kernel<DIST, 8, 8>},
    {16, 8, infer_heads_kernel<DIST, 16, 8>}};
template <class E, size_t C>
static const E* heads_pick(const E (&tab)[C], int K, int A) {
  for (const E& e : tab)
    if (K / 32 <= e.kpl && A <= e.amax) return &e;
  return nullptr;
}
static bool heads_fit(int K, int A, bool infer = false) {
  return K % 32 == 0 && (infer ? heads_pick(kInferHeadsKernels<Categorical>, K, A) != nullptr
                               : heads_pick(kHeadsKernels<PpoLoss>, K, A) != nullptr);
}

static cudaError_t ensure_kernel_attrs() {
  static bool done = false;
  if (done) return cudaSuccess;
  cudaError_t e = cudaSuccess;
  auto opt_in = [&](const void* k) { if (e == cudaSuccess) e = cudaFuncSetAttribute(k, cudaFuncAttributeMaxDynamicSharedMemorySize, kMaxDynSmem); };
  for (auto k : kRowsKernels<0>) opt_in((const void*)k);
  for (auto k : kRowsKernels<1>) opt_in((const void*)k);
  for (auto k : kRowsKernels<2>) opt_in((const void*)k);
  for (auto k : kWgradKernels) opt_in((const void*)k);
  for (const auto& h : kHeadsKernels<PpoLoss>) opt_in((const void*)h.kern);
  for (const auto& h : kHeadsKernels<DuelingTdLoss>) opt_in((const void*)h.kern);
  for (const auto& h : kHeadsKernels<PpoGaussLoss>) opt_in((const void*)h.kern);
  done = e == cudaSuccess;
  return e;
}

template <int KIND>
static cudaError_t launch_rows(bp::RowsArgs& a, cudaStream_t st) {
  const auto kern = by_width(kRowsKernels<KIND>, a.N);
  if (!kern) return cudaErrorInvalidValue;
  { cudaError_t e0 = ensure_kernel_attrs(); if (e0 != cudaSuccess) return e0; }
  const int epi_planes = KIND == 2 ? bp::dgrad_epi_planes(a.src_act, a.accumulate) : 0;
  const RowsSmem m = rows_smem(a.w_res != 0, a.w_res_chunks, a.w_pitch, a.mode, (size_t)a.n_stage_ents, (size_t)a.n_units, a.N,
                               epi_planes);
  if (m.n_stages < 2) return cudaErrorInvalidConfiguration;
  const int smem = 128 + m.wres_bytes + m.n_stages * m.stage_bytes + m.epi_banks * m.epi_bank_bytes + m.tab_bytes;
  const int total = a.n_units * a.n_btiles;
  const int grid = std::min(total, kSMs);
  XLAUNCH(kern, grid, bp::RW_THREADS, smem, st, a, m.n_stages, m.stage_bytes, m.wres_bytes, m.epi_banks);
  return cudaPeekAtLastError();
}

static cudaError_t launch_wgrad(const bp::WgradArgs& a, int grid, cudaStream_t st) {
  const auto kern = by_width(kWgradKernels, a.N);
  if (!kern) return cudaErrorInvalidValue;
  { cudaError_t e0 = ensure_kernel_attrs(); if (e0 != cudaSuccess) return e0; }
  const size_t smem = wgrad_smem(a.mode, a.n_opix, a.R);
  if (smem > (size_t)kMaxDynSmem) return cudaErrorInvalidConfiguration;
  XLAUNCH(kern, grid, bp::WG_THREADS, (int)smem, st, a);
  return cudaPeekAtLastError();
}

static void queue_reduction(xtb_net* net, const float* part, int n_slabs, long long slab, int count, long long dst_off,
                            float* dst_ptr = nullptr, const LayerPlan* conv = nullptr) {
  bp::RedSeg r;
  memset(&r, 0, sizeof r);
  r.part = part; r.n_slabs = n_slabs; r.slab = slab; r.count = count; r.kind = conv ? 0 : 1;
  r.dst_off = dst_off; r.dst_ptr = dst_ptr; r.alpha = 1.f;
  if (conv) {
    r.N = conv->N; r.C = conv->q.C; r.KW = conv->q.KW; r.mts = conv->mts; r.s2d_k4 = conv->s2d ? conv->k4 : 0;
    r.alpha = conv->d.src == 0 ? net->desc.scale : 1.f;
  }
  net->pending.push_back(r);
}

static cudaError_t tc_forward(xtb_net* net, int i, int B, int split_rows, bool want_f32, bool want_bp, cudaStream_t st,
                              long long* launches) {
  const LayerPlan& lp = net->L[i];
  const int t = i + 1;
  bp::RowsArgs a;
  memset(&a, 0, sizeof a);
  a.a = lp.d.src == 0 ? obs_bp(net) : out_bp(net, lp.d.src);
  a.a_split = lp.d.src != 0;
  a.w_hi = blob_hi(net, lp); a.w_lo = a.w_hi + net->blob_elems; a.w_pitch = lp.K;
  a.B = B; a.n_btiles = (B + 127) / 128; a.N = lp.n_fwd;
  const bool ext = act_is_ext(lp.d.act);
  a.out = want_bp && !ext ? out_bp(net, t) : no_bp();
  a.out_f32 = ext ? pre_buf(net, t) : (want_f32 ? out_f32(net, t) : nullptr);
  a.ld_f32 = net->tsize[t];
  a.bias = net->params + lp.b_off;
  a.alpha = lp.d.src == 0 ? net->desc.scale : 1.f;
  a.act = ext ? 0 : lp.d.act;
  *launches = 1;
  if (lp.d.kind == XTB_CONV) {
    a.mode = 0;
    a.stages = (const bp::StageEnt*)(net->ws + lp.fwd_st_off); a.units = (const bp::UnitEnt*)(net->ws + lp.fwd_un_off);
    a.n_stage_ents = (int)lp.fwd_st.size();
    a.w_res = lp.w_res; a.w_res_chunks = lp.N / 8;
    a.n_units = lp.q.OH * lp.q.OW;
    return launch_rows<0>(a, st);
  }
  a.mode = 2;
  a.kchunks = lp.K / 8; a.n_ntiles = lp.N / lp.n_fwd;
  const DenseSplit sp = dense_split(lp, B, split_rows);
  const int nz = sp.nz;
  a.kc_split = sp.kc_split;
  a.n_units = a.n_ntiles * nz;
  if (nz == 1) return launch_rows<0>(a, st);
  a.part = (float*)(net->ws + net->splitk_off);
  const int b_pad = (B + 15) & ~15;
  a.part_z = (long long)b_pad * lp.N; a.ld_part = lp.N;
  cudaError_t e = launch_rows<1>(a, st);
  if (e != cudaSuccess) return e;
  long long pieces = (long long)(lp.N / 8) * b_pad * bp::FIN_ZL;
  XLAUNCH(bp::bp_splitk_finish_kernel, (unsigned)((pieces + 127) / 128), 128, 0, st, (const float*)a.part, nz, a.part_z, B, lp.N,
          a.bias, a.act, a.out_f32, a.out);
  *launches = 2;
  return cudaPeekAtLastError();
}

static cudaError_t tc_dgrad(xtb_net* net, int i, int B, int accumulate, float* db_part, cudaStream_t st) {
  const LayerPlan& lp = net->L[i];
  const int t = i + 1, s = lp.d.src;
  bp::RowsArgs a;
  memset(&a, 0, sizeof a);
  a.a = gout_bp(net, t); a.a_split = 1;
  a.w_hi = blob_hi(net, lp); a.w_lo = a.w_hi + net->blob_elems; a.w_pitch = lp.K;
  a.B = B; a.n_btiles = (B + 127) / 128; a.N = lp.n_dg;
  a.out = gout_bp(net, s); a.src = out_bp(net, s); a.src_act = dgrad_act(lp); a.accumulate = accumulate; a.db_part = db_part;
  if (lp.d.kind == XTB_CONV) {
    a.mode = 1;
    a.stages = (const bp::StageEnt*)(net->ws + lp.dg_st_off); a.units = (const bp::UnitEnt*)(net->ws + lp.dg_un_off);
    a.n_stage_ents = (int)lp.dg_st.size();
    a.w_res = lp.w_res; a.w_res_chunks = lp.N / 8;
    a.n_units = lp.q.H * lp.q.W;
  } else {
    a.mode = 2;
    a.kchunks = lp.N / 8; a.kc_split = a.kchunks; a.n_ntiles = lp.K / lp.n_dg;
    a.n_units = a.n_ntiles;
  }
  return launch_rows<2>(a, st);
}

static cudaError_t tc_wgrad(xtb_net* net, int i, int B, cudaStream_t st) {
  LayerPlan& lp = net->L[i];
  const int t = i + 1;
  bp::WgradArgs a;
  memset(&a, 0, sizeof a);
  a.x = lp.d.src == 0 ? obs_bp(net) : out_bp(net, lp.d.src);
  a.x_split = lp.d.src != 0;
  a.g = gout_bp(net, t);
  a.zeros = (const bp::bf16*)(net->ws + net->zeros_off);
  a.B = B; a.n_bsub = (B + bp::WG_KB - 1) / bp::WG_KB;
  if (lp.d.kind == XTB_CONV) {
    const ConvGeom& q = lp.q;
    a.mode = 0;
    a.tab = (const bp::WgEnt*)(net->ws + lp.wg_off);
    a.R = lp.R; a.N = lp.N; a.n_opix = q.OH * q.OW; a.n_ntiles = 1;
    a.part = (float*)(net->ws + lp.part_off);
    const int slices = std::max(1, std::min(kSMs / lp.R, a.n_opix * a.n_bsub));
    queue_reduction(net, a.part, slices, (long long)lp.R * 128 * lp.N, lp.R * 128 * lp.N, lp.w_off, nullptr, &lp);
    return launch_wgrad(a, lp.R * slices, st);
  }
  a.mode = 1;
  a.N = std::min(lp.n_fwd, 64);
  a.x_chunks = lp.K / 8; a.r_tiles = (lp.K + 127) / 128; a.n_ntiles = lp.N / a.N; a.n_opix = 1; a.R = 1;
  a.dw = net->grads + lp.w_off; a.ldw = lp.N; a.k_rows = lp.K;
  return launch_wgrad(a, std::min(kSMs, a.r_tiles * a.n_ntiles), st);
}

extern "C" int xtb_net_sync_weights(xtb_net* net, void* stream) {
  if (!net || !net->ws || !net->params) return fail(XTB_ERR_STATE, "xtb_net_sync_weights: net not bound");
  if (net->blob_segs.empty()) return XTB_OK;
  long long mx = 0;
  for (const auto& s : net->blob_segs) mx = std::max(mx, (long long)(s.N / 8) * s.K);
  dim3 grid((unsigned)((mx + 127) / 128), (unsigned)net->blob_segs.size());
  XLAUNCH(bp::bp_wprep_kernel, grid, 128, 0, S(stream), (const float*)net->params, (const bp::BlobSeg*)(net->ws + net->segs_off),
          (bp::bf16*)(net->ws + net->blob_off), net->blob_elems);
  LAUNCH_CHECK();
  return XTB_OK;
}


static int ensure_bp(xtb_net* net, int t, int B, bool grad, cudaStream_t st) {
  const uint8_t f = forms(net, t, grad);
  if (f & kPlanes) return XTB_OK;
  if (!(f & kF32)) return fail(XTB_ERR_STATE, "tensor %d has no current %s", t, grad ? "gradient" : "value");
  const float* src = grad ? gout_f32(net, t) : out_f32(net, t);
  const int F = net->tsize[t], b_pad = (B + 15) & ~15;
  long long pieces = (long long)(F / 8) * b_pad;
  XLAUNCH(bp::bp_split_kernel, (unsigned)((pieces + 127) / 128), 128, 0, st, src, B, F, grad ? gout_bp(net, t) : out_bp(net, t));
  LAUNCH_CHECK();
  wrote(net, t, grad, kBoth);
  return XTB_OK;
}
static int ensure_f32(xtb_net* net, int t, int B, bool grad, cudaStream_t st) {
  const uint8_t f = forms(net, t, grad);
  if (f & kF32) return XTB_OK;
  if (!(f & kPlanes)) return fail(XTB_ERR_STATE, "tensor %d has no current %s", t, grad ? "gradient" : "value");
  float* dst = grad ? gout_f32(net, t) : out_f32(net, t);
  const int F = net->tsize[t];
  long long pieces = (long long)(F / 8) * B;
  XLAUNCH(bp::bp_merge_kernel, (unsigned)((pieces + 127) / 128), 128, 0, st, grad ? gout_bp(net, t) : out_bp(net, t), B, F, dst);
  LAUNCH_CHECK();
  wrote(net, t, grad, kBoth);
  return XTB_OK;
}

extern "C" int xtb_tc_gemm_test(int mode, const float* a, const float* b, float* c, int M, int N, int K, int ksplit,
                                void* stream) {
  if (!a || !b || !c || M <= 0 || N <= 0 || K <= 0) return fail(XTB_ERR_ARG, "xtb_tc_gemm_test: bad argument");
  if (N % 16 || K % 16 || (mode == 2 && M % 16)) return fail(XTB_ERR_ARG, "xtb_tc_gemm_test: N, K (and M for mode 2) must be multiples of 16");
  cudaStream_t st = S(stream);
  const int rows = mode == 2 ? K : M;
  const int pitch = (rows + 15) / 16 * 16;
  const int fa = mode == 2 ? M : K;
  const int fb = N;
  const int nt = pick_tile(N);
  if (!nt) return fail(XTB_ERR_ARG, "N must be a multiple of 16");
  bp::bf16 *pa = nullptr, *pw = nullptr, *pc = nullptr; float* part = nullptr; float* bias = nullptr;
  const long long ea = (long long)fa * pitch;
  const long long ew = mode == 2 ? (long long)fb * pitch : (mode == 1 ? (long long)K * ((N + 15) / 16 * 16) : (long long)N * K);
  const long long ec = (long long)N * pitch;
  CUDA_TRY(cudaMalloc(&pa, 2 * ea * sizeof(bp::bf16)));
  CUDA_TRY(cudaMalloc(&pw, 2 * ew * sizeof(bp::bf16) + 256));
  CUDA_TRY(cudaMalloc(&pc, 2 * ec * sizeof(bp::bf16) + 4096));
  CUDA_TRY(cudaMalloc(&bias, (size_t)std::max(N, 64) * sizeof(float)));
  CUDA_TRY(cudaMemsetAsync(pa, 0, 2 * ea * sizeof(bp::bf16), st));
  CUDA_TRY(cudaMemsetAsync(pw, 0, 2 * ew * sizeof(bp::bf16) + 256, st));
  CUDA_TRY(cudaMemsetAsync(pc, 0, 2 * ec * sizeof(bp::bf16) + 4096, st));
  CUDA_TRY(cudaMemsetAsync(bias, 0, (size_t)std::max(N, 64) * sizeof(float), st));
  bp::BpT ta{pa, ea, pitch}, tw{pw, ew, mode == 2 ? pitch : K}, tcp{pc, ec, pitch};
  auto split = [&](const float* src, int B_, int F_, bp::BpT dst) {
    long long pieces = (long long)(F_ / 8) * ((B_ + 15) & ~15);
    XLAUNCH(bp::bp_split_kernel, (unsigned)((pieces + 127) / 128), 128, 0, st, src, B_, F_, dst);
  };
  cudaError_t e = cudaSuccess;
  if (mode == 0 || mode == 1) {
    split(a, M, K, ta);
    if (mode == 0) { tw.pitch = K; split(b, K, N, tw); }
    else { tw.pitch = (N + 15) / 16 * 16; split(b, N, K, tw); }
    bp::RowsArgs r;
    memset(&r, 0, sizeof r);
    r.a = ta; r.a_split = 1; r.w_hi = pw; r.w_lo = pw + ew; r.w_pitch = tw.pitch;
    r.mode = 2; r.B = M; r.n_btiles = (M + 127) / 128; r.N = nt; r.n_ntiles = N / nt;
    r.kchunks = K / 8; r.kc_split = r.kchunks;
    r.bias = bias; r.alpha = 1.f; r.act = 0;
    if (mode == 0) {
      int nz = 1;
      if (ksplit > 1) { r.kc_split = ((r.kchunks + ksplit - 1) / ksplit + 7) / 8 * 8; nz = (r.kchunks + r.kc_split - 1) / r.kc_split; }
      r.n_units = r.n_ntiles * nz;
      if (nz > 1) {
        CUDA_TRY(cudaMalloc(&part, (size_t)nz * M * N * sizeof(float)));
        r.part = part; r.part_z = (long long)M * N; r.ld_part = N;
        e = launch_rows<1>(r, st);
        long long pieces = (long long)(N / 8) * ((M + 15) & ~15) * bp::FIN_ZL;
        XLAUNCH(bp::bp_splitk_finish_kernel, (unsigned)((pieces + 127) / 128), 128, 0, st, (const float*)part, nz, r.part_z, M, N,
                (const float*)bias, 0, c, no_bp());
      } else {
        r.out_f32 = c; r.ld_f32 = N;
        e = launch_rows<0>(r, st);
      }
    } else {
      r.n_units = r.n_ntiles;
      r.out = tcp; r.src = tcp; r.src_act = 0;
      e = launch_rows<2>(r, st);
      long long pieces = (long long)(N / 8) * M;
      XLAUNCH(bp::bp_merge_kernel, (unsigned)((pieces + 127) / 128), 128, 0, st, tcp, M, N, c);
    }
  } else {
    split(a, K, M, ta);
    split(b, K, N, tw);
    bp::WgradArgs w;
    memset(&w, 0, sizeof w);
    w.x = ta; w.x_split = 1; w.g = tw; w.zeros = pc;
    w.mode = 1; w.N = nt; w.B = K; w.n_bsub = (K + bp::WG_KB - 1) / bp::WG_KB; w.n_opix = 1; w.R = 1;
    w.x_chunks = M / 8; w.r_tiles = (M + 127) / 128; w.n_ntiles = N / nt;
    w.dw = c; w.ldw = N; w.k_rows = M;
    e = launch_wgrad(w, std::min(kSMs, w.r_tiles * w.n_ntiles), st);
  }
  g_launches.fetch_add(4, std::memory_order_relaxed);
  cudaError_t e2 = cudaStreamSynchronize(st);
  cudaFree(pa); cudaFree(pw); cudaFree(pc); cudaFree(bias); cudaFree(part);
  if (e != cudaSuccess) return fail(XTB_ERR_CUDA, "tc gemm launch: %s", cudaGetErrorString(e));
  if (e2 != cudaSuccess) return fail(XTB_ERR_CUDA, "tc gemm run: %s", cudaGetErrorString(e2));
  return XTB_OK;
}

template <typename T>
static void conv_fwd(const LayerPlan& lp, const T* x, const int32_t* idx, const float* w, const float* b,
                     float alpha, float* out, int B, cudaStream_t st) {
  int M = B * lp.g.P;
  BRowMajor bl{w, lp.N};
  EpiBiasAct ep{out, b, alpha, act_is_ext(lp.d.act) ? 0 : lp.d.act, lp.N, nullptr, 0};
  if (lp.pad) { AIm2col<T, true> al{x, idx, lp.g, lp.koff, lp.kyx}; launch_gemm(al, bl, ep, M, lp.N, lp.K, false, st); }
  else { AIm2col<T, false> al{x, idx, lp.g, lp.koff, lp.kyx}; launch_gemm(al, bl, ep, M, lp.N, lp.K, false, st); }
}
template <typename T>
static void dense_fwd(const LayerPlan& lp, const T* x, const int32_t* idx, const float* w, const float* b,
                      float alpha, float* out, int B, cudaStream_t st) {
  ADense<T> al{x, idx, lp.K};
  BRowMajor bl{w, lp.N};
  EpiBiasAct ep{out, b, alpha, act_is_ext(lp.d.act) ? 0 : lp.d.act, lp.N, nullptr, 0};
  launch_gemm(al, bl, ep, B, lp.N, lp.K, false, st);
}
template <typename T>
static void conv_wgrad(const LayerPlan& lp, const T* x, const int32_t* idx, const float* dy, float alpha,
                       float* dw, int B, cudaStream_t st, bool bias_row = true) {
  int Mr = B * lp.g.P;
  BRowMajor bl{dy, lp.N};
  EpiAtomic ep{dw, alpha, lp.N};
  int rows = lp.K + ((alpha == 1.f && bias_row) ? 1 : 0);
  if (lp.pad) { AIm2colT<T, true> al{x, idx, lp.g, lp.koff, lp.kyx, Mr}; launch_gemm(al, bl, ep, rows, lp.N, Mr, true, st); }
  else { AIm2colT<T, false> al{x, idx, lp.g, lp.koff, lp.kyx, Mr}; launch_gemm(al, bl, ep, rows, lp.N, Mr, true, st); }
}
template <typename T>
static void dense_wgrad(const LayerPlan& lp, const T* x, const int32_t* idx, const float* dy, float alpha,
                        float* dw, int B, cudaStream_t st, bool bias_row = true) {
  ADenseT<T> al{x, idx, lp.K, lp.K};
  BRowMajor bl{dy, lp.N};
  EpiAtomic ep{dw, alpha, lp.N};
  launch_gemm(al, bl, ep, lp.K + ((alpha == 1.f && bias_row) ? 1 : 0), lp.N, B, true, st);
}

__global__ void colsum_kernel(const float* __restrict__ dy, int M, int N, float* __restrict__ db) {
  pdl_wait(); pdl_trigger();
  int n = blockIdx.x * 32 + (threadIdx.x & 31);
  int r0 = blockIdx.y * 1024 + (threadIdx.x >> 5);
  float s = 0.f;
  if (n < N)
    for (int m = r0; m < min(M, (int)(blockIdx.y + 1) * 1024); m += 8) s += dy[(long long)m * N + n];
  __shared__ float red[8][33];
  red[threadIdx.x >> 5][threadIdx.x & 31] = s;
  __syncthreads();
  if (threadIdx.x < 32 && n < N) {
    float t = 0.f;
    for (int i = 0; i < 8; i++) t += red[i][threadIdx.x];
    atomicAdd(db + n, t);
  }
}

static int act_forward(xtb_net* net, int t, int B, cudaStream_t st) {
  const long long n = (long long)B * net->tsize[t];
  const unsigned blocks = (unsigned)std::min<long long>((n + 255) / 256, 8LL * kSMs);
  XLAUNCH(act_fwd_kernel, blocks, 256, 0, st, (const float*)pre_buf(net, t), n, net->L[t - 1].d.act, out_f32(net, t));
  LAUNCH_CHECK();
  wrote(net, t, false, kF32);
  return XTB_OK;
}
static int act_backward(xtb_net* net, int t, int B, cudaStream_t st) {
  int rc = ensure_f32(net, t, B, true, st);
  if (rc) return rc;
  const LayerPlan& lp = net->L[t - 1];
  const float* u = z_buf(net, t) ? z_buf(net, t) : out_f32(net, t);
  float* part = (float*)(net->ws + lp.act_part_off);
  XLAUNCH(act_bwd_kernel, ACT_BWD_BLOCKS, ACT_BWD_THREADS, 0, st, gout_f32(net, t), u,
          (int)((long long)B * net->tsize[t] / lp.N), lp.N, lp.d.act, part);
  LAUNCH_CHECK();
  queue_reduction(net, part, ACT_BWD_BLOCKS, lp.N, lp.N, lp.b_off);
  wrote(net, t, true, kF32);
  return XTB_OK;
}

static int op_decode(xtb_net* net, const void* obs, const int32_t* idx, int B, cudaStream_t st) {
  if (forms(net, 0, false) & kPlanes) return XTB_OK;
  const LayerPlan* first = nullptr;
  for (const auto& lp : net->L) if (lp.s2d && use_tc(lp)) { first = &lp; break; }
  if (!first) return XTB_OK;
  dim3 grid(4 * net->H4, (B + bp::DEC_SAMPLES - 1) / bp::DEC_SAMPLES);
  const int smem = bp::DEC_SAMPLES * (net->desc.in_w * 4 + 8);
  XLAUNCH(bp::bp_decode_s2d_kernel, grid, bp::DEC_THREADS, smem, st, (const uint8_t*)obs, idx, B, net->desc.in_h, net->desc.in_w, net->H4,
          net->W4, first->g.padT, first->g.padL, net->desc.input_u8 == 2 ? 1 : 0, obs_bp(net));
  LAUNCH_CHECK();
  wrote(net, 0, false, kPlanes);
  return XTB_OK;
}

template <class F>
static void with_obs_type(const xtb_net* net, const void* obs, F&& f) {
  if (net->desc.input_u8 == 2) f((const int8_t*)obs);
  else if (net->desc.input_u8) f((const uint8_t*)obs);
  else f((const float*)obs);
}

static int op_forward(xtb_net* net, int i, const float* P, bool tc_allowed, const void* obs, const int32_t* idx, int B,
                      int split_rows, bool want_f32, cudaStream_t st) {
  const LayerPlan& lp = net->L[i];
  const int t = i + 1;
  float* out = out_f32(net, t);
  const bool ext = act_is_ext(lp.d.act);
  float* pre = ext ? pre_buf(net, t) : out;
  const float* w = P + lp.w_off;
  const float* b = P + lp.b_off;
  if (lp.d.kind == XTB_LOGSTD) return XTB_OK;
  if (lp.d.kind == XTB_DUELING) {
    int rc = ensure_f32(net, lp.d.src, B, false, st);
    if (!rc) rc = ensure_f32(net, lp.d.k, B, false, st);
    if (rc) return rc;
    XLAUNCH(dueling_fwd_kernel, (B + 7) / 8, 256, 0, st, (const float*)out_f32(net, lp.d.src), (const float*)out_f32(net, lp.d.k), B,
            lp.out_size, out);
    LAUNCH_CHECK();
    wrote(net, t, false, kF32);
    return XTB_OK;
  }
  if (tc_allowed && use_tc(lp)) {
    int rc = lp.d.src == 0 ? op_decode(net, obs, idx, B, st) : ensure_bp(net, lp.d.src, B, false, st);
    if (rc) return rc;
    long long nl = 0;
    cudaError_t te = tc_forward(net, i, B, split_rows, want_f32, true, st, &nl);
    if (te != cudaSuccess) return fail(XTB_ERR_CUDA, "tensor-core forward launch (layer %d): %s", i, cudaGetErrorString(te));
    g_launches.fetch_add(nl, std::memory_order_relaxed);
    if (ext) return act_forward(net, t, B, st);
    wrote(net, t, false, want_f32 ? kBoth : kPlanes);
    return XTB_OK;
  }
  auto gemm = [&](auto x, const int32_t* ix, float alpha) {
    if (lp.d.kind == XTB_CONV) conv_fwd(lp, x, ix, w, b, alpha, pre, B, st);
    else dense_fwd(lp, x, ix, w, b, alpha, pre, B, st);
  };
  if (lp.d.src == 0) {
    with_obs_type(net, obs, [&](auto x) { gemm(x, idx, net->desc.scale); });
  } else {
    int rc = ensure_f32(net, lp.d.src, B, false, st);
    if (rc) return rc;
    gemm((const float*)out_f32(net, lp.d.src), nullptr, 1.f);
  }
  LAUNCH_CHECK();
  if (ext) return act_forward(net, t, B, st);
  wrote(net, t, false, kF32);
  return XTB_OK;
}

static int op_wgrad(xtb_net* net, int i, const void* obs, const int32_t* idx, int B, cudaStream_t st, bool bias_done = false) {
  const LayerPlan& lp = net->L[i];
  if (lp.d.kind == XTB_DUELING || lp.d.kind == XTB_LOGSTD) return XTB_OK;
  int t = i + 1;
  float* dw = net->grads + lp.w_off;
  float* db = net->grads + lp.b_off;
  const bool tc = use_tc(lp);
  if (tc) {
    int rc = ensure_bp(net, t, B, true, st);
    if (rc) return rc;
    rc = lp.d.src == 0 ? op_decode(net, obs, idx, B, st) : ensure_bp(net, lp.d.src, B, false, st);
    if (rc) return rc;
    cudaError_t te = tc_wgrad(net, i, B, st);
    if (te != cudaSuccess) return fail(XTB_ERR_CUDA, "tensor-core wgrad launch (layer %d): %s", i, cudaGetErrorString(te));
  } else {
    int rc = ensure_f32(net, t, B, true, st);
    if (rc) return rc;
    const float* dy = gout_f32(net, t);
    auto gemm = [&](auto x, const int32_t* ix, float alpha) {
      if (lp.d.kind == XTB_CONV) conv_wgrad(lp, x, ix, dy, alpha, dw, B, st, !bias_done);
      else dense_wgrad(lp, x, ix, dy, alpha, dw, B, st, !bias_done);
    };
    if (lp.d.src == 0) {
      with_obs_type(net, obs, [&](auto x) { gemm(x, idx, net->desc.scale); });
    } else {
      rc = ensure_f32(net, lp.d.src, B, false, st);
      if (rc) return rc;
      gemm((const float*)out_f32(net, lp.d.src), nullptr, 1.f);
    }
  }
  LAUNCH_CHECK();
  if (bias_done || (!tc && (lp.d.src != 0 || net->desc.scale == 1.f))) return XTB_OK;
  if (forms(net, t, true) & kF32) {
    int Mb = lp.d.kind == XTB_CONV ? B * lp.g.P : B;
    dim3 gridb((lp.N + 31) / 32, (Mb + 1023) / 1024);
    XLAUNCH(colsum_kernel, gridb, 256, 0, st, (const float*)gout_f32(net, t), Mb, lp.N, db);
  } else {
    XLAUNCH(bp::bp_colsum_kernel, (net->tsize[t] / 8 + 3) / 4, 128, 0, st, gout_bp(net, t), B, net->tsize[t], lp.N, db);
  }
  LAUNCH_CHECK();
  return XTB_OK;
}

static int op_dgrad(xtb_net* net, int i, int acc, int B, cudaStream_t st, bool fuse_db = false, int acc2 = 0) {
  const LayerPlan& lp = net->L[i];
  int t = i + 1, s = lp.d.src;
  if (lp.d.kind == XTB_DUELING) {
    const int s2 = lp.d.k;
    int rc = ensure_f32(net, t, B, true, st);
    if (!rc) rc = ensure_f32(net, s, B, false, st);
    if (!rc) rc = ensure_f32(net, s2, B, false, st);
    if (!rc && acc) rc = ensure_f32(net, s, B, true, st);
    if (!rc && acc2) rc = ensure_f32(net, s2, B, true, st);
    if (rc) return rc;
    XLAUNCH(dueling_dgrad_kernel, (B + 7) / 8, 256, 0, st, (const float*)gout_f32(net, t), (const float*)out_f32(net, s),
            (const float*)out_f32(net, s2), B, lp.out_size, lp.src_act, lp.adv_act, acc, acc2, gout_f32(net, s), gout_f32(net, s2));
    LAUNCH_CHECK();
    wrote(net, s, true, kF32); wrote(net, s2, true, kF32);
    return XTB_OK;
  }
  if (use_tc(lp)) {
    int rc = ensure_bp(net, t, B, true, st);
    if (rc) return rc;
    if (dgrad_act(lp) != 0) { rc = ensure_bp(net, s, B, false, st); if (rc) return rc; }
    if (acc) { rc = ensure_bp(net, s, B, true, st); if (rc) return rc; }
    float* dbp = fuse_db ? (float*)(net->ws + lp.dbpart_off) : nullptr;
    cudaError_t te = tc_dgrad(net, i, B, acc, dbp, st);
    if (te != cudaSuccess) return fail(XTB_ERR_CUDA, "tensor-core dgrad launch (layer %d): %s", i, cudaGetErrorString(te));
    LAUNCH_CHECK();
    if (fuse_db) {
      const int units = lp.d.kind == XTB_CONV ? lp.q.H * lp.q.W : lp.K / lp.n_dg;
      queue_reduction(net, dbp, std::min(kSMs, units * ((B + 127) / 128)), lp.n_dg, lp.n_dg, net->L[s - 1].b_off);
    }
    wrote(net, s, true, kPlanes);
    return XTB_OK;
  }
  int rc = ensure_f32(net, t, B, true, st);
  if (rc) return rc;
  rc = ensure_f32(net, s, B, false, st);
  if (rc) return rc;
  if (acc) { rc = ensure_f32(net, s, B, true, st); if (rc) return rc; }
  const float* dy = gout_f32(net, t);
  const float* x = out_f32(net, s);
  float* gsrc = gout_f32(net, s);
  const float* w = net->params + lp.w_off;
  if (lp.d.kind == XTB_CONV) {
    ADgrad al{dy, lp.g, lp.dkyx, lp.dco, lp.sshift};
    BConvDgrad bl{w, lp.wk, lp.N};
    EpiDgrad ep{gsrc, x, dgrad_act(lp), lp.g.C, acc, nullptr, 0};
    launch_gemm(al, bl, ep, B * lp.g.H * lp.g.W, lp.g.C, lp.Kd, false, st);
  } else {
    ADense<float> al{dy, nullptr, lp.N};
    BTransposed bl{w, lp.N};
    EpiDgrad ep{gsrc, x, dgrad_act(lp), lp.K, acc, nullptr, 0};
    launch_gemm(al, bl, ep, B, lp.K, lp.N, false, st);
  }
  LAUNCH_CHECK();
  wrote(net, s, true, kF32);
  return XTB_OK;
}

static int flush_reductions(xtb_net* net, cudaStream_t st) {
  if (net->pending.empty()) return XTB_OK;
  bp::RedSegs segs;
  memset(&segs, 0, sizeof segs);
  int mx = 0;
  if (net->pending.size() > bp::RED_MAX) return fail(XTB_ERR_STATE, "too many pending reductions");
  for (size_t k = 0; k < net->pending.size(); k++) { segs.s[k] = net->pending[k]; mx = std::max(mx, net->pending[k].count); }
  dim3 grid((mx + 127) / 128, (unsigned)net->pending.size());
  XLAUNCH(bp::grad_reduce_kernel, grid, 256, 0, st, segs, net->grads);
  LAUNCH_CHECK();
  net->pending.clear();
  return XTB_OK;
}

static int net_forward_impl(xtb_net* net, const float* params, const void* obs, const int32_t* gather_idx,
                            int batch, void* stream, unsigned skip_mask, unsigned want_f32_mask, int split_rows = 0);
extern "C" int xtb_net_forward(xtb_net* net, const float* params, const void* obs, const int32_t* gather_idx,
                               int batch, void* stream) {
  return net_forward_impl(net, params, obs, gather_idx, batch, stream, 0u, ~0u);
}
static int net_forward_impl(xtb_net* net, const float* params, const void* obs, const int32_t* gather_idx,
                            int batch, void* stream, unsigned skip_mask, unsigned want_f32_mask, int split_rows) {
  if (!net || !net->ws) return fail(XTB_ERR_STATE, "xtb_net_forward: net not bound");
  if (batch <= 0 || batch > net->max_batch) return fail(XTB_ERR_ARG, "batch %d out of range (max %d)", batch, net->max_batch);
  if (!obs) return fail(XTB_ERR_ARG, "obs is null");
  const float* P = params ? params : net->params;
  const bool tc_allowed = (P == net->params);
  cudaStream_t st = S(stream);
  const int nl = (int)net->L.size();
  invalidate(net, true, false);
  for (int i = 0; i < nl; i++) {
    if (skip_mask & (1u << i)) continue;
    const LayerPlan& lp = net->L[i];
    bool direct = lp.d.kind == XTB_DENSE && ((want_f32_mask >> (i + 1)) & 1u);
    if (lp.d.kind == XTB_DENSE)
      for (int j = i + 1; j < nl; j++)
        if (reads(net->L[j], i + 1) && !(skip_mask & (1u << j)) && !(tc_allowed && use_tc(net->L[j]))) direct = true;
    int rc = op_forward(net, i, P, tc_allowed, obs, gather_idx, batch, split_rows ? split_rows : batch, direct, st);
    if (rc) return rc;
  }
  for (int t = 1; t <= nl; t++) {
    if (!((want_f32_mask >> t) & 1u) || (skip_mask & (1u << (t - 1))) || net->tsize[t] == 0) continue;
    int rc = ensure_f32(net, t, batch, false, st);
    if (rc) return rc;
  }
  return XTB_OK;
}

struct BackwardOpts {
  const int32_t* heads; int n_heads;
  unsigned heads_bp = 0u;
  unsigned heads_dy = 0u;
  unsigned skip = 0u;
  bool zero_grads = true;
  unsigned bias_done = 0u;
  float* dobs = nullptr;
  bool all_reduce = false;
  BackwardOpts(const int32_t* h, int n) : heads(h), n_heads(n) {}
};
static int net_backward_impl(xtb_net* net, const void* obs, const int32_t* gather_idx, int batch, void* stream,
                             const BackwardOpts& o);
extern "C" int xtb_net_backward(xtb_net* net, const void* obs, const int32_t* gather_idx, int batch,
                                const int32_t* head_tensors, int n_heads, void* stream) {
  return net_backward_impl(net, obs, gather_idx, batch, stream, BackwardOpts(head_tensors, n_heads));
}
static int input_grad_check(const xtb_net* net) {
  if (net->desc.input_u8 || net->desc.scale != 1.f) return fail(XTB_ERR_ARG, "input gradient: the observation must be float with scale 1");
  for (const auto& lp : net->L)
    if (lp.d.src == 0 && lp.d.kind != XTB_DENSE && lp.d.kind != XTB_LOGSTD)
      return fail(XTB_ERR_ARG, "input gradient: only dense layers may read the observation");
  return XTB_OK;
}
extern "C" int xtb_net_backward_input(xtb_net* net, const void* obs, const int32_t* gather_idx, int batch,
                                      const int32_t* head_tensors, int n_heads, float* dobs, void* stream) {
  if (!obs || !dobs || !head_tensors) return fail(XTB_ERR_ARG, "xtb_net_backward_input: null pointer");
  BackwardOpts o(head_tensors, n_heads); o.dobs = dobs;
  return net_backward_impl(net, obs, gather_idx, batch, stream, o);
}
static int net_backward_impl(xtb_net* net, const void* obs, const int32_t* gather_idx, int batch, void* stream,
                             const BackwardOpts& o) {
  if (!net || !net->ws || !net->grads) return fail(XTB_ERR_STATE, "xtb_net_backward: net not bound (grads required)");
  if (batch <= 0 || batch > net->max_batch) return fail(XTB_ERR_ARG, "batch out of range");
  if (o.dobs) { int rc = input_grad_check(net); if (rc) return rc; }
  cudaStream_t st = S(stream);
  xtb_comm* comm = o.all_reduce ? g_comm : nullptr;
  const int nl = (int)net->L.size();
  std::vector<char> has_grad(nl + 1, 0), written(nl + 1, 0);
  std::vector<char> dy(nl + 1, 0);
  long long early_off = 0, early_cnt = 0;
  invalidate(net, false, true);
  if (o.zero_grads) net->pending.clear();
  for (int h = 0; h < o.n_heads; h++) {
    int t = o.heads[h];
    if (t < 1 || t > nl || net->tsize[t] == 0) return fail(XTB_ERR_ARG, "bad head tensor %d", t);
    has_grad[t] = 1; written[t] = 1; dy[t] = (o.heads_dy >> t) & 1u;
    wrote(net, t, true, (o.heads_bp >> t) & 1u ? kPlanes : kF32);
  }
  if (o.zero_grads) CUDA_TRY(cudaMemsetAsync(net->grads, 0, net->n_params * sizeof(float), st));
  std::vector<char> fuse_bias(nl + 1, 0);
  for (int s = 1; s <= nl; s++) {
    if (o.bias_done & (1u << s)) { fuse_bias[s] = 2; continue; }
    const LayerPlan& ps = net->L[s - 1];
    if (act_is_ext(ps.d.act)) continue;
    int consumers = 0, cj = -1;
    for (int j = 0; j < nl; j++) if (reads(net->L[j], s) && !(o.skip & (1u << j))) { consumers++; cj = j; }
    if (consumers != 1) continue;
    const LayerPlan& c = net->L[cj];
    if (!use_tc(c)) continue;
    if (ps.d.kind == XTB_CONV ? c.n_dg == ps.N : (c.d.kind == XTB_DENSE && c.n_dg == ps.N && c.K == ps.N)) fuse_bias[s] = 1;
  }
  for (int i = nl - 1; i >= 0; i--) {
    if (o.skip & (1u << i)) continue;
    const LayerPlan& lp = net->L[i];
    int t = i + 1;
    if (!has_grad[t]) continue;
    const bool act_bwd = dy[t] && act_is_ext(lp.d.act);
    if (act_bwd) { int rc = act_backward(net, t, batch, st); if (rc) return rc; }
    int rc = op_wgrad(net, i, obs, gather_idx, batch, st, fuse_bias[t] != 0 || act_bwd);
    if (rc) return rc;
    if (comm && comm->world > 1 && early_cnt == 0 && lp.d.kind == XTB_DENSE && use_tc(lp) && (long long)lp.K * lp.N >= (1 << 16)) {
      early_off = lp.w_off; early_cnt = (long long)lp.K * lp.N;
      rc = comm_fork_allreduce(comm, net->grads + early_off, early_cnt, st);
      if (rc) return rc;
    }
    if (lp.d.kind == XTB_DUELING) {
      const int s = lp.d.src, s2 = lp.d.k;
      rc = op_dgrad(net, i, written[s] ? 1 : 0, batch, st, false, written[s2] ? 1 : 0);
      if (rc) return rc;
      written[s] = written[s2] = 1; has_grad[s] = has_grad[s2] = 1;
    } else if (lp.d.src != 0) {
      int s = lp.d.src;
      rc = op_dgrad(net, i, written[s] ? 1 : 0, batch, st, fuse_bias[s] == 1);
      if (rc) return rc;
      written[s] = 1; has_grad[s] = 1; dy[s] = 1;
    }
  }
  if (o.dobs) {
    bool first = true;
    for (int i = 0; i < nl; i++) {
      const LayerPlan& lp = net->L[i];
      if (lp.d.src != 0 || lp.d.kind != XTB_DENSE || (o.skip & (1u << i))) continue;
      if (!has_grad[i + 1]) continue;
      int rc = ensure_f32(net, i + 1, batch, true, st);
      if (rc) return rc;
      ADense<float> al{(const float*)gout_f32(net, i + 1), nullptr, lp.N};
      BTransposed bl{net->params + lp.w_off, lp.N};
      EpiDgrad ep{o.dobs, o.dobs, 0, lp.K, first ? 0 : 1, nullptr, 0};
      launch_gemm(al, bl, ep, batch, lp.K, lp.N, false, st);
      LAUNCH_CHECK();
      first = false;
    }
    if (first) CUDA_TRY(cudaMemsetAsync(o.dobs, 0, (size_t)batch * net->tsize[0] * sizeof(float), st));
  }
  int rc = flush_reductions(net, st);
  if (rc || !comm || comm->world == 1) return rc;
  if (early_cnt == 0) return xtb_comm_allreduce(comm, net->grads, net->n_params, stream);
  int nrc = g_nccl.GroupStart();
  if (!nrc && early_off > 0) nrc = g_nccl.AllReduce(net->grads, net->grads, (size_t)early_off, kNcclFloat, kNcclSum, comm->comm, st);
  const long long tail = net->n_params - (early_off + early_cnt);
  if (!nrc && tail > 0)
    nrc = g_nccl.AllReduce(net->grads + early_off + early_cnt, net->grads + early_off + early_cnt, (size_t)tail, kNcclFloat, kNcclSum, comm->comm, st);
  int erc = g_nccl.GroupEnd();
  if (nrc || erc) return fail(XTB_ERR_CUDA, "ncclAllReduce: %s", g_nccl.GetErrorString(nrc ? nrc : erc));
  return comm_join(comm, st);
}

extern "C" int xtb_net_bench_layer(xtb_net* net, int layer, int which, const void* obs, const int32_t* gather_idx,
                                   int batch, void* stream) {
  if (!net || !net->ws || !net->grads) return fail(XTB_ERR_STATE, "xtb_net_bench_layer: net not bound");
  if (layer < 0 || layer >= (int)net->L.size() || batch <= 0 || batch > net->max_batch) return fail(XTB_ERR_ARG, "bad layer/batch");
  cudaStream_t st = S(stream);
  for (int t = 1; t <= (int)net->L.size(); t++)
    for (bool grad : {false, true})
      if (forms(net, t, grad) == kNone) wrote(net, t, grad, kF32);
  if (which == 0) return op_forward(net, layer, net->params, true, obs, gather_idx, batch, batch, false, st);
  if (which == 1) { int rc = op_wgrad(net, layer, obs, gather_idx, batch, st, true); net->pending.clear(); return rc; }
  if (which == 2) {
    if (net->L[layer].d.src == 0) return fail(XTB_ERR_ARG, "layer reads the observation: no data gradient");
    int rc = op_dgrad(net, layer, 0, batch, st);
    net->pending.clear();
    return rc;
  }
  if (which == 3) { wrote(net, 0, false, kNone); return op_decode(net, obs, gather_idx, batch, st); }
  return fail(XTB_ERR_ARG, "xtb_net_bench_layer: which must be 0..3");
}


extern "C" int xtb_categorical_sample(const float* logits, int batch, int adim, const float* uniforms,
                                      uint64_t seed, uint64_t offset, int32_t* action, float* logp, void* stream) {
  if (!logits || !action || !logp || batch <= 0 || adim <= 0) return fail(XTB_ERR_ARG, "xtb_categorical_sample: bad argument");
  XLAUNCH(sample_kernel<Categorical>, (batch + 127) / 128, 128, 0, S(stream), logits, (const float*)nullptr, batch, batch, adim,
          uniforms, seed, offset, (const unsigned long long*)nullptr, 0, action, logp, (const float*)nullptr, (float*)nullptr);
  LAUNCH_CHECK();
  return XTB_OK;
}

extern "C" int xtb_argmax(const float* q, int batch, int adim, int32_t* action, void* stream) {
  if (!q || !action || batch <= 0 || adim <= 0) return fail(XTB_ERR_ARG, "xtb_argmax: bad argument");
  XLAUNCH(argmax_kernel, (batch + 127) / 128, 128, 0, S(stream), q, batch, adim, action);
  LAUNCH_CHECK();
  return XTB_OK;
}

extern "C" int xtb_gae(const float* value, const float* reward, const uint8_t* done, int n_env, int n_step,
                       float gamma, float lam, int sign_clip, float* adv, float* old_value, float* target_value,
                       void* stream) {
  if (!value || !reward || !done || !adv || !old_value || !target_value) return fail(XTB_ERR_ARG, "xtb_gae: null pointer");
  if (n_env == 0 || n_step == 0) return XTB_OK;
  if (n_env < 0 || n_step < 0) return fail(XTB_ERR_ARG, "xtb_gae: negative size");
  int threads = 128;
  int blocks = (n_env * 32 + threads - 1) / threads;
  XLAUNCH(gae_kernel, blocks, threads, 0, S(stream), value, reward, done, n_env, n_step, gamma, lam, sign_clip, adv,
                                                old_value, target_value);
  LAUNCH_CHECK();
  return XTB_OK;
}

extern "C" int xtb_ppo_loss_grad(const float* logits, const float* v, const int32_t* gather_idx,
                                 const int32_t* action, const float* old_logp, const float* adv,
                                 const float* old_v, const float* target_v, int batch, int adim,
                                 const xtb_ppo_hyper* hp, float inv_count, float* dlogits, float* dv,
                                 float* loss_out, void* stream) {
  if (!logits || !v || !action || !old_logp || !adv || !old_v || !target_v || !hp || !dlogits || !dv || !loss_out)
    return fail(XTB_ERR_ARG, "xtb_ppo_loss_grad: null pointer");
  if (batch <= 0 || adim <= 0 || adim > MAX_ADIM) return fail(XTB_ERR_ARG, "xtb_ppo_loss_grad: batch/adim out of range");
  PpoHyperDev h{hp->clip_ratio, hp->ent_coef, hp->vf_clip, hp->critic_coef};
  XLAUNCH(ppo_loss_kernel, (batch + 127) / 128, 128, 0, S(stream), logits, v, gather_idx, action, old_logp, adv, old_v,
                                                              target_v, batch, adim, h, inv_count, dlogits, dv, loss_out);
  LAUNCH_CHECK();
  return XTB_OK;
}

extern "C" int xtb_diag_gaussian_sample(const float* mean, const float* log_std, int batch, int adim, const float* normals,
                                        uint64_t seed, uint64_t offset, float* action, float* logp, void* stream) {
  if (!mean || !log_std || !action || !logp || batch <= 0 || adim <= 0 || adim > MAX_ADIM)
    return fail(XTB_ERR_ARG, "xtb_diag_gaussian_sample: bad argument");
  XLAUNCH(sample_kernel<DiagGaussian>, (batch + 127) / 128, 128, 0, S(stream), mean, log_std, batch, batch, adim, normals, seed,
          offset, (const unsigned long long*)nullptr, 0, action, logp, (const float*)nullptr, (float*)nullptr);
  LAUNCH_CHECK();
  return XTB_OK;
}

extern "C" int xtb_ppo_gauss_loss_grad(const float* mean, const float* v, const float* log_std, const int32_t* gather_idx,
                                       const float* action, const float* old_logp, const float* adv, const float* old_v,
                                       const float* target_v, int batch, int adim, const xtb_ppo_hyper* hp, float inv_count,
                                       float* dmean, float* dv, float* dlog_std, float* loss_out, void* stream) {
  if (!mean || !v || !log_std || !action || !old_logp || !adv || !old_v || !target_v || !hp || !dmean || !dv || !dlog_std || !loss_out)
    return fail(XTB_ERR_ARG, "xtb_ppo_gauss_loss_grad: null pointer");
  if (batch <= 0 || adim <= 0 || adim > MAX_ADIM) return fail(XTB_ERR_ARG, "xtb_ppo_gauss_loss_grad: batch/adim out of range");
  PpoHyperDev h{hp->clip_ratio, hp->ent_coef, hp->vf_clip, hp->critic_coef};
  if (adim <= 8)
    XLAUNCH(ppo_gauss_loss_kernel<8>, 1, GAUSS_LOSS_THREADS, 0, S(stream), mean, v, log_std, gather_idx, action, old_logp, adv, old_v,
            target_v, batch, adim, h, inv_count, dmean, dv, dlog_std, loss_out);
  else
    XLAUNCH(ppo_gauss_loss_kernel<MAX_ADIM>, 1, GAUSS_LOSS_THREADS, 0, S(stream), mean, v, log_std, gather_idx, action, old_logp, adv,
            old_v, target_v, batch, adim, h, inv_count, dmean, dv, dlog_std, loss_out);
  LAUNCH_CHECK();
  return XTB_OK;
}

extern "C" int xtb_vtrace_loss_grad(const float* tp_logits, const float* baseline, const float* bp_logits,
                                    const int32_t* action, const uint8_t* done, const float* reward,
                                    int n_traj, int step_len, int adim, float gamma, float* dlogits,
                                    float* dbaseline, float* vs_out, float* pg_adv_out, float* loss_out,
                                    void* stream) {
  if (!tp_logits || !baseline || !bp_logits || !action || !done || !reward || !dlogits || !dbaseline || !loss_out)
    return fail(XTB_ERR_ARG, "xtb_vtrace_loss_grad: null pointer");
  if (n_traj <= 0 || step_len < 2 || adim <= 0 || adim > MAX_ADIM) return fail(XTB_ERR_ARG, "xtb_vtrace_loss_grad: bad sizes");
  int threads = 128;
  int blocks = (n_traj * 32 + threads - 1) / threads;
  XLAUNCH(vtrace_kernel, blocks, threads, 0, S(stream), tp_logits, baseline, bp_logits, action, done, reward, n_traj,
                                                   step_len, adim, gamma, dlogits, dbaseline, vs_out, pg_adv_out, loss_out);
  LAUNCH_CHECK();
  return XTB_OK;
}

extern "C" int xtb_dqn_td_loss_grad(const float* q, const float* q_next_target, const float* q_next_online, const int32_t* idx,
                                    const int32_t* action, const float* reward, const uint8_t* done, const float* disc, int batch,
                                    int adim, float gamma, float huber_delta, float inv_count, float* dq, float* y_out,
                                    float* loss_out, void* stream) {
  if (!q || !q_next_target || !action || !reward || !done || !dq || !loss_out) return fail(XTB_ERR_ARG, "xtb_dqn_td_loss_grad: null pointer");
  if (batch <= 0 || adim <= 0) return fail(XTB_ERR_ARG, "xtb_dqn_td_loss_grad: bad sizes");
  XLAUNCH(dqn_loss_kernel, (batch + 127) / 128, 128, 0, S(stream), q, q_next_target, q_next_online, idx, action, reward, done, disc,
          batch, adim, gamma, huber_delta, inv_count, dq, y_out, loss_out);
  LAUNCH_CHECK();
  return XTB_OK;
}
extern "C" int xtb_dqn_loss_grad(const float* q, const float* q_next_target, const float* q_next_online,
// ... 82 lines not shown
    for (long long b = seg[s]; b < seg[s + 1]; b += OPT_CHUNK) {
      bseg.push_back(s); bbeg.push_back(b); blen.push_back((int)std::min<long long>(OPT_CHUNK, seg[s + 1] - b));
    }
  o->n_blk = (int)bseg.size();
  AdamState init{1.f, 1.f, 0.f, 0.f, 0u};
  cudaError_t e = cudaSuccess;
  auto chk = [&](cudaError_t r) { if (e == cudaSuccess) e = r; };
  chk(cudaMalloc(&o->blk_seg, o->n_blk * sizeof(int)));
  chk(cudaMalloc(&o->blk_beg, o->n_blk * sizeof(long long)));
  chk(cudaMalloc(&o->blk_len, o->n_blk * sizeof(int)));
  chk(cudaMalloc(&o->norm_sq, o->n_seg * sizeof(double)));
  chk(cudaMalloc(&o->seg_scale, o->n_seg * sizeof(float)));
  chk(cudaMalloc(&o->st, sizeof(AdamState)));
  chk(cudaMalloc(&o->hyp, sizeof(AdamHyper)));
  chk(cudaMalloc(&o->ticket, sizeof(unsigned int)));
  if (e == cudaSuccess) {
    chk(cudaMemcpy(o->blk_seg, bseg.data(), o->n_blk * sizeof(int), cudaMemcpyHostToDevice));
    chk(cudaMemcpy(o->blk_beg, bbeg.data(), o->n_blk * sizeof(long long), cudaMemcpyHostToDevice));
    chk(cudaMemcpy(o->blk_len, blen.data(), o->n_blk * sizeof(int), cudaMemcpyHostToDevice));
    chk(cudaMemset(o->norm_sq, 0, o->n_seg * sizeof(double)));
    chk(cudaMemcpy(o->st, &init, sizeof init, cudaMemcpyHostToDevice));
    chk(cudaMemset(o->ticket, 0, sizeof(unsigned int)));
    AdamHyper hy{lr, beta1, beta2, eps, clip, 0.f};
    chk(cudaMemcpy(o->hyp, &hy, sizeof hy, cudaMemcpyHostToDevice));
    chk(cudaMemset(m, 0, count * sizeof(float)));
    chk(cudaMemset(v, 0, count * sizeof(float)));
  }
  if (e != cudaSuccess) { xtb_adam_destroy(o); return fail(XTB_ERR_CUDA, "xtb_adam_create: %s", cudaGetErrorString(e)); }
  *out = o;
  return XTB_OK;
}

extern "C" void xtb_adam_destroy(xtb_adam* o) {
  if (!o) return;
  drop_graphs_of(o);
  cudaFree(o->blk_seg); cudaFree(o->blk_beg); cudaFree(o->blk_len);
  cudaFree(o->norm_sq); cudaFree(o->seg_scale); cudaFree(o->st); cudaFree(o->hyp); cudaFree(o->ticket);
  delete o;
}

static int adam_step_impl(xtb_adam* o, float* params, const float* grads, float grad_scale, void* stream, xtb_net* net);
extern "C" int xtb_adam_step(xtb_adam* o, float* params, const float* grads, float grad_scale, void* stream) {
  return adam_step_impl(o, params, grads, grad_scale, stream, nullptr);
}
extern "C" int xtb_adam_step_net(xtb_adam* o, xtb_net* net, float grad_scale, void* stream) {
  if (!net || !net->ws || !net->params || !net->grads) return fail(XTB_ERR_STATE, "xtb_adam_step_net: net not bound");
  if (!o || o->count != net->n_params) return fail(XTB_ERR_ARG, "xtb_adam_step_net: optimiser/net size mismatch");
  return adam_step_impl(o, net->params, net->grads, grad_scale, stream, net);
}
static int adam_step_impl(xtb_adam* o, float* params, const float* grads, float grad_scale, void* stream, xtb_net* net) {
  if (!o || !params || !grads) return fail(XTB_ERR_ARG, "xtb_adam_step: null pointer");
  if (misaligned16(params) || misaligned16(grads) || misaligned16(o->m) || misaligned16(o->v) || misaligned16(o->mg))
    return fail(XTB_ERR_ARG, "xtb_adam_step: params, grads and the optimiser slots must be 16-byte aligned");
  cudaStream_t st = S(stream);
  XLAUNCH(sqnorm_kernel, (o->n_blk + SQN_GROUP - 1) / SQN_GROUP, OPT_THREADS, 0, st, grads, o->blk_seg, o->blk_beg, o->blk_len, o->n_blk, o->norm_sq, o->ticket, o->st,
          (const AdamHyper*)o->hyp, o->seg_scale, o->n_seg, o->clip_mode, grad_scale);
  LAUNCH_CHECK();
  const bool blobs = net && !net->blob_segs.empty();
  if (o->mg || o->rms_plain) {
    XLAUNCH(o->mg ? rmsprop_kernel<true> : rmsprop_kernel<false>, o->n_blk, OPT_THREADS, 0, st, params, grads, o->m, o->mg, o->blk_seg, o->blk_beg, o->blk_len,
            o->seg_scale, (const AdamHyper*)o->hyp, o->rms_rho, o->rms_eps, blobs ? (const bp::BlobSeg*)(net->ws + net->segs_off) : nullptr,
            blobs ? (int)net->blob_segs.size() : 0, blobs ? (__nv_bfloat16*)(net->ws + net->blob_off) : nullptr, blobs ? net->blob_elems : 0LL);
    LAUNCH_CHECK();
    return XTB_OK;
  }
  XLAUNCH(adam_kernel, o->n_blk, OPT_THREADS, 0, st, params, grads, o->m, o->v, o->blk_seg, o->blk_beg, o->blk_len,
          o->seg_scale, o->st, (const AdamHyper*)o->hyp, blobs ? (const bp::BlobSeg*)(net->ws + net->segs_off) : nullptr,
          blobs ? (int)net->blob_segs.size() : 0, blobs ? (__nv_bfloat16*)(net->ws + net->blob_off) : nullptr, blobs ? net->blob_elems : 0LL);
  LAUNCH_CHECK();
  return XTB_OK;
}

extern "C" const float* xtb_adam_grad_norm(const xtb_adam* o) { return o ? &o->st->grad_norm : nullptr; }
extern "C" int xtb_opt_use_rmsprop(xtb_adam* o, float* mean_grad, float decay, float epsilon) {
  if (!o || !mean_grad) return fail(XTB_ERR_ARG, "xtb_opt_use_rmsprop: null pointer");
  if (misaligned16(mean_grad)) return fail(XTB_ERR_ARG, "xtb_opt_use_rmsprop: mean_grad must be 16-byte aligned");
  if (!(decay > 0.f && decay < 1.f) || !(epsilon > 0.f)) return fail(XTB_ERR_ARG, "xtb_opt_use_rmsprop: decay in (0,1), epsilon > 0");
  drop_graphs_of(o);
  {
    std::vector<float> ones((size_t)o->count, 1.f);
    CUDA_TRY(cudaDeviceSynchronize());
    CUDA_TRY(cudaMemcpy(o->m, ones.data(), ones.size() * sizeof(float), cudaMemcpyHostToDevice));
    CUDA_TRY(cudaMemset(mean_grad, 0, ones.size() * sizeof(float)));
  }
  o->mg = mean_grad; o->rms_rho = decay; o->rms_eps = epsilon; o->rms_plain = false;
  return XTB_OK;
}
extern "C" int xtb_opt_use_rmsprop_plain(xtb_adam* o, float decay, float epsilon) {
  if (!o) return fail(XTB_ERR_ARG, "xtb_opt_use_rmsprop_plain: null pointer");
  if (!(decay > 0.f && decay < 1.f) || !(epsilon > 0.f)) return fail(XTB_ERR_ARG, "xtb_opt_use_rmsprop_plain: decay in (0,1), epsilon > 0");
  drop_graphs_of(o);
  {
    std::vector<float> ones((size_t)o->count, 1.f);
    CUDA_TRY(cudaDeviceSynchronize());
    CUDA_TRY(cudaMemcpy(o->m, ones.data(), ones.size() * sizeof(float), cudaMemcpyHostToDevice));
  }
  o->mg = nullptr; o->rms_rho = decay; o->rms_eps = epsilon; o->rms_plain = true;
  return XTB_OK;
}
extern "C" int xtb_adam_set_lr(xtb_adam* o, float lr) {
  if (!o) return fail(XTB_ERR_ARG, "null optimiser");
  o->lr = lr;
  CUDA_TRY(cudaDeviceSynchronize());
  CUDA_TRY(cudaMemcpy(&o->hyp->lr, &lr, sizeof lr, cudaMemcpyHostToDevice));
  return XTB_OK;
}
extern "C" int xtb_adam_set_decay(xtb_adam* o, float decay) {
  if (!o) return fail(XTB_ERR_ARG, "null optimiser");
  if (!(decay >= 0.f)) return fail(XTB_ERR_ARG, "xtb_adam_set_decay: decay must be >= 0");
  CUDA_TRY(cudaDeviceSynchronize());
  CUDA_TRY(cudaMemcpy(&o->hyp->decay, &decay, sizeof decay, cudaMemcpyHostToDevice));
  return XTB_OK;
}

struct EngineStream { cudaStream_t st = nullptr; cudaEvent_t in = nullptr, out = nullptr; };
static EngineStream g_engine_streams[64];
struct StreamScope {
  cudaStream_t st = nullptr;
  EngineStream* es = nullptr;
  int begin(void* stream, bool side_if_null) {
    st = S(stream);
    if (st || !side_if_null) return XTB_OK;
    int dev = 0;
    CUDA_TRY(cudaGetDevice(&dev));
    if (dev < 0 || dev >= 64) return fail(XTB_ERR_ARG, "device index %d out of range", dev);
    EngineStream& e = g_engine_streams[dev];
    if (!e.st) {
      CUDA_TRY(cudaStreamCreateWithFlags(&e.st, cudaStreamNonBlocking));
      CUDA_TRY(cudaEventCreateWithFlags(&e.in, cudaEventDisableTiming));
      CUDA_TRY(cudaEventCreateWithFlags(&e.out, cudaEventDisableTiming));
    }
    CUDA_TRY(cudaEventRecord(e.in, nullptr));
    CUDA_TRY(cudaStreamWaitEvent(e.st, e.in, 0));
    es = &e; st = e.st;
    return XTB_OK;
  }
  int end() {
    if (!es) return XTB_OK;
    CUDA_TRY(cudaEventRecord(es->out, es->st));
    CUDA_TRY(cudaStreamWaitEvent(nullptr, es->out, 0));
    es = nullptr;
    return XTB_OK;
  }
};
static int g_fuse_heads = [] { const char* e = getenv("XTB_FUSE_HEADS"); return e ? atoi(e) : 1; }();
extern "C" int xtb_set_fuse_heads(int on) { g_fuse_heads = on; return XTB_OK; }

enum GraphTag { kPpoTrain = 1, kImpalaTrain, kDqnTrain, kRolloutInfer, kImpalaKerasFit, kImpalaKerasTrain, kMuzeroTrain,
                kMuzeroInitInfer, kMuzeroRecurInfer, kMuzeroSearch, kQmixTrain, kQmixInfer,
                kSccTrain, kSccInfer, kSccCritic };
struct CaptureKey {
  uint64_t tag;
  const void* own[6];
  uint64_t mode[2];
  uint64_t arg[21];
  bool operator<(const CaptureKey& o) const { return memcmp(this, &o, sizeof(CaptureKey)) < 0; }
};
template <class T> static uint64_t key_word(T v) {
  if constexpr (std::is_same_v<T, float>) { uint32_t u; memcpy(&u, &v, sizeof u); return u; }
  else if constexpr (std::is_same_v<T, double>) { uint64_t u; memcpy(&u, &v, sizeof u); return u; }
  else if constexpr (std::is_pointer_v<T>) return (uint64_t)(uintptr_t)v;
  else return (uint64_t)v;
}
template <size_t N, class... A>
static CaptureKey capture_key(GraphTag tag, const void* const (&owners)[N], A... args) {
  static_assert(N < sizeof(CaptureKey::own) / sizeof(void*), "CaptureKey::own too small");
  static_assert(sizeof...(A) <= sizeof(CaptureKey::arg) / sizeof(uint64_t), "CaptureKey::arg too small");
  CaptureKey k;
  memset(&k, 0, sizeof k);
  k.tag = tag;
  std::copy(owners, owners + N, k.own);
  const uint64_t w[] = {key_word(args)...};
  memcpy(k.arg, w, sizeof w);
  return k;
}
struct GraphVal { cudaGraphExec_t exec; long long kernels; };
static constexpr size_t kMaxCachedGraphs = 256;
static std::map<CaptureKey, GraphVal> g_graphs;
static std::atomic<long long> g_graph_replays{0};
extern "C" long long xtb_graph_replay_count(void) { return g_graph_replays.load(); }

static void drop_graphs_of(const void* obj) {
  for (auto it = g_graphs.begin(); it != g_graphs.end();) {
    const auto& own = it->first.own;
    if (std::find(std::begin(own), std::end(own), obj) != std::end(own)) { cudaGraphExecDestroy(it->second.exec); it = g_graphs.erase(it); } else ++it;
  }
}

template <class F>
static int run_graph(CaptureKey key, int use_graph, void* stream, F&& launch) {
  if (!use_graph) return launch(stream);
  key.own[5] = g_comm; key.mode[0] = g_tc_mode; key.mode[1] = g_fuse_heads;
  StreamScope sc;
  int src = sc.begin(stream, true);
  if (src) return src;
  auto it = g_graphs.find(key);
  if (it == g_graphs.end()) {
    cudaStream_t st = sc.st;
    long long before = g_launches.load();
    CUDA_TRY(cudaStreamBeginCapture(st, cudaStreamCaptureModeThreadLocal));
    int rc = launch((void*)st);
    cudaGraph_t graph = nullptr;
    cudaError_t e = cudaStreamEndCapture(st, &graph);
    long long captured = g_launches.load() - before;
    g_launches.store(before);
    if (rc) { if (graph) cudaGraphDestroy(graph); return rc; }
    if (e != cudaSuccess) return fail(XTB_ERR_CUDA, "graph capture failed: %s", cudaGetErrorString(e));
    cudaGraphExec_t exec = nullptr;
    e = cudaGraphInstantiate(&exec, graph, 0);
    cudaGraphDestroy(graph);
    if (e != cudaSuccess) return fail(XTB_ERR_CUDA, "graph instantiate failed: %s", cudaGetErrorString(e));
    if (g_graphs.size() >= kMaxCachedGraphs) {
      for (auto& kv : g_graphs) cudaGraphExecDestroy(kv.second.exec);
      g_graphs.clear();
    }
    it = g_graphs.emplace(key, GraphVal{exec, captured}).first;
  }
  CUDA_TRY(cudaGraphLaunch(it->second.exec, sc.st));
  g_launches.fetch_add(it->second.kernels, std::memory_order_relaxed);
  g_graph_replays.fetch_add(1, std::memory_order_relaxed);
  return sc.end();
}

template <class STEP>
static int ppo_epoch_loop(xtb_net* net, xtb_adam* opt, int N, int B, int E, const int32_t* perm, float* loss_per_step,
                          void* stream, STEP&& minibatch) {
  int steps_per_epoch = (N + B - 1) / B;
  CUDA_TRY(cudaMemsetAsync(loss_per_step, 0, sizeof(float) * E * steps_per_epoch, S(stream)));
  int step = 0;
  for (int e = 0; e < E; e++) {
    for (int s0 = 0; s0 < N; s0 += B, step++) {
      int mb = std::min(B, N - s0);
      int rc = minibatch(perm + (long long)e * N + s0, mb, loss_per_step + step);
      if (rc) return rc;
      rc = xtb_adam_step_net(opt, net, 1.f, stream);
      if (rc) return rc;
    }
  }
  return XTB_OK;
}

static float dp_inv_world() { return g_comm ? 1.f / g_comm->world : 1.f; }

static int learner_check(const char* fn, bool missing, const xtb_net* net, const xtb_adam* opt, long long rows, bool dp_ok,
                         long long max_rows = 0, long long n_params = 0) {
  if (missing) return fail(XTB_ERR_ARG, "%s: null pointer", fn);
  if (!net->ws || !net->grads) return fail(XTB_ERR_STATE, "%s: net not bound", fn);
  if (!dp_ok && g_comm) return fail(XTB_ERR_STATE, "%s: data-parallel training (communicator) is not supported", fn);
  if (opt && opt->count != (n_params ? n_params : net->n_params))
    return fail(XTB_ERR_ARG, "%s: optimiser/net size mismatch (%lld != %lld)", fn, opt->count, n_params ? n_params : net->n_params);
  if (!max_rows) max_rows = net->max_batch;
  if (rows < 1 || rows > max_rows) return fail(XTB_ERR_ARG, "%s: batch %lld not in [1, %lld]", fn, rows, max_rows);
  return XTB_OK;
}

static bool ppo_heads_fusable(const xtb_net* net, int pi_t, int v_t, bool infer) {
  const LayerPlan& lpi = net->L[pi_t - 1];
  const LayerPlan& lv = net->L[v_t - 1];
  return g_fuse_heads && lpi.d.kind == XTB_DENSE && lv.d.kind == XTB_DENSE && lpi.d.act == 0 && lv.d.act == 0 &&
         lpi.d.src != 0 && lv.d.src != 0 && lpi.K == lv.K && heads_fit(lpi.K, net->tsize[pi_t], infer);
}

template <class LOSS>
static int heads_fused(xtb_net* net, const void* obs, PpoHeadsArgs& a, int mb, int pi_t, int v_t, unsigned skip,
                       long long ls_off, float* loss_dst, void* stream) {
  const LayerPlan& lpi = net->L[pi_t - 1];
  const LayerPlan& lv = net->L[v_t - 1];
  const int adim = net->tsize[pi_t];
  const int32_t* idx = a.idx;
  CUDA_TRY(cudaMemsetAsync(net->grads, 0, net->n_params * sizeof(float), S(stream)));
  net->pending.clear();
  a.h_pi = out_f32(net, lpi.d.src); a.h_v = out_f32(net, lv.d.src);
  a.g_pi = gout_f32(net, lpi.d.src); a.g_v = gout_f32(net, lv.d.src);
  const bool ext_pi = act_is_ext(lpi.src_act), ext_v = act_is_ext(lv.src_act);
  const bool bp_pi = use_tc(net->L[lpi.d.src - 1]) && net->plane_elems[lpi.d.src] > 0 && !ext_pi;
  const bool bp_v = use_tc(net->L[lv.d.src - 1]) && net->plane_elems[lv.d.src] > 0 && !ext_v;
  a.gp_hi = bp_pi ? gout_bp(net, lpi.d.src).hi : nullptr; a.gp_lo = net->plane_elems[lpi.d.src];
  a.gv_hi = bp_v ? gout_bp(net, lv.d.src).hi : nullptr; a.gv_lo = net->plane_elems[lv.d.src];
  a.pitch = net->pitch;
  a.w_pi = net->params + lpi.w_off; a.b_pi = net->params + lpi.b_off; a.w_v = net->params + lv.w_off; a.b_v = net->params + lv.b_off;
  auto only_feeds_heads = [&](int tsr) { for (int j = 0; j < (int)net->L.size(); j++) if (reads(net->L[j], tsr) && !(skip & (1u << j))) return false; return true; };
  bool bh_pi_ok = net->L[lpi.d.src - 1].d.kind == XTB_DENSE && only_feeds_heads(lpi.d.src) && !ext_pi;
  bool bh_v_ok = net->L[lv.d.src - 1].d.kind == XTB_DENSE && only_feeds_heads(lv.d.src) && !ext_v;
  a.B = mb; a.K = lpi.K; a.A = adim; a.act_pi = dgrad_act(lpi); a.act_v = dgrad_act(lv); a.shared = lpi.d.src == lv.d.src ? 1 : 0;
  int blocks = std::max(1, std::min(kSMs, (mb + 7) / 8));
  const int HK = lpi.K, nacc = HK * adim + 3 * HK + adim + 2 + (LOSS::kLogStd ? adim : 0);
  a.part = (float*)(net->ws + net->heads_part_off); a.slab = (nacc + 3) & ~3;
  size_t shb = (size_t)8 * nacc * sizeof(float);
  { cudaError_t ea = ensure_kernel_attrs(); if (ea != cudaSuccess) return fail(XTB_ERR_CUDA, "kernel attributes: %s", cudaGetErrorString(ea)); }
  XLAUNCH(heads_pick(kHeadsKernels<LOSS>, a.K, a.A)->kern, blocks, 256, shb, S(stream), a);
  LAUNCH_CHECK();
  {
    auto seg = [&](int off, int count, long long dst_off, float* dst_ptr = nullptr) {
      queue_reduction(net, a.part + off, blocks, a.slab, count, dst_off, dst_ptr);
    };
    seg(0, HK * adim, lpi.w_off);
    seg(HK * adim, HK, lv.w_off);
    if (bh_pi_ok) seg(HK * adim + HK, HK, net->L[lpi.d.src - 1].b_off);
    if (!a.shared && bh_v_ok) seg(HK * adim + 2 * HK, HK, net->L[lv.d.src - 1].b_off);
    seg(HK * adim + 3 * HK, adim, lpi.b_off);
    seg(HK * adim + 3 * HK + adim, 1, lv.b_off);
    seg(HK * adim + 3 * HK + adim + 1, 1, 0, loss_dst);
    if (LOSS::kLogStd) seg(HK * adim + 3 * HK + adim + 2, adim, ls_off);
  }
  const int32_t srcs[2] = {lpi.d.src, lv.d.src};
  BackwardOpts o(srcs, a.shared ? 1 : 2);
  o.heads_bp = (bp_pi ? (1u << lpi.d.src) : 0u) | (bp_v ? (1u << lv.d.src) : 0u);
  o.heads_dy = (ext_pi ? (1u << lpi.d.src) : 0u) | (ext_v ? (1u << lv.d.src) : 0u);
  o.bias_done = (bh_pi_ok ? (1u << lpi.d.src) : 0u) | ((lpi.d.src != lv.d.src && bh_v_ok) ? (1u << lv.d.src) : 0u);
  o.skip = skip; o.zero_grads = false; o.all_reduce = true;
  return net_backward_impl(net, obs, idx, mb, stream, o);
}

template <class DIST>
static int ppo_train_launch(xtb_net* net, xtb_adam* opt, const xtb_ppo_rollout* ro, int N, int B, int E, const int32_t* perm,
                            const xtb_ppo_hyper* hp, int pi_t, int v_t, int ls_t, float* loss_per_step, float inv_world,
                            void* stream) {
  const int32_t heads[2] = {pi_t, v_t};
  const auto* action = static_cast<const typename DIST::Action*>(ro->action);
  const int adim = net->tsize[pi_t];
  const long long ls_off = DIST::kLogStd ? net->L[ls_t - 1].w_off : -1;
  const LayerPlan& lpi = net->L[pi_t - 1];
  const LayerPlan& lv = net->L[v_t - 1];
  const bool fuse = ppo_heads_fusable(net, pi_t, v_t, false);
  const unsigned skip = fuse ? ((1u << (pi_t - 1)) | (1u << (v_t - 1))) : 0u;
  return ppo_epoch_loop(net, opt, N, B, E, perm, loss_per_step, stream, [&](const int32_t* idx, int mb, float* step_loss) -> int {
    const unsigned want = fuse ? ((1u << lpi.d.src) | (1u << lv.d.src)) : ((1u << pi_t) | (1u << v_t));
    int rc = net_forward_impl(net, nullptr, ro->obs, idx, mb, stream, skip, want);
    if (rc) return rc;
    if (fuse) {
      PpoHeadsArgs a;
      memset(&a, 0, sizeof a);
      a.idx = idx; a.old_logp = ro->old_logp; a.adv = ro->adv; a.old_v = ro->old_v; a.target_v = ro->target_v;
      if constexpr (DIST::kLogStd) { a.action_f = action; a.log_std = net->params + ls_off; }
      else a.action = action;
      a.logits_out = xtb_net_tensor(net, pi_t); a.v_out = xtb_net_tensor(net, v_t);
      a.hp = PpoHyperDev{hp->clip_ratio, hp->ent_coef, hp->vf_clip, hp->critic_coef}; a.inv_count = inv_world / mb;
      return heads_fused<typename DIST::Loss>(net, ro->obs, a, mb, pi_t, v_t, skip, ls_off, step_loss, stream);
    }
    if constexpr (DIST::kLogStd) {
      CUDA_TRY(cudaMemsetAsync(net->grads, 0, net->n_params * sizeof(float), S(stream)));
      rc = xtb_ppo_gauss_loss_grad(xtb_net_tensor(net, pi_t), xtb_net_tensor(net, v_t), net->params + ls_off, idx, action,
                                   ro->old_logp, ro->adv, ro->old_v, ro->target_v, mb, adim, hp, inv_world / mb,
                                   xtb_net_tensor_grad(net, pi_t), xtb_net_tensor_grad(net, v_t), net->grads + ls_off, step_loss,
                                   stream);
    } else {
      rc = xtb_ppo_loss_grad(xtb_net_tensor(net, pi_t), xtb_net_tensor(net, v_t), idx, action, ro->old_logp, ro->adv,
                             ro->old_v, ro->target_v, mb, adim, hp, inv_world / mb, xtb_net_tensor_grad(net, pi_t),
// ... 1120 lines not shown
```

Measured before the change: 288,700.

## Overlap weight-gradient GEMMs with data-gradient GEMMs on a side stream

Small backward layers now launch their weight-gradient GEMM on a per-device side stream, forked and joined with events, so it can run concurrently with the data-gradient GEMM of the same layer. Eligibility is decided by a stage-count heuristic. To make sharing the GPU possible, the rows and wgrad kernels are reworked to iterate over virtual CTAs, with an optional cap on the physical grid size, and the dbias partial is flushed per virtual CTA. This adds stream and event overhead inside graph capture and risks contention between the overlapped kernels.

```diff
diff --git a/include/xtb200.h b/include/xtb200.h
--- a/include/xtb200.h
+++ b/include/xtb200.h
@@ -296,6 +296,8 @@
 
 int xtb_set_tc_mode(int mode);
 int xtb_set_fuse_heads(int on);
+int xtb_set_bwd_overlap(int mode);
+int xtb_set_gemm_cta_cap(int cap);
 int xtb_get_tc_mode(void);
 int xtb_tc_gemm_test(int mode, const float* a, const float* b, float* c, int M, int N, int K, int ksplit,
                      void* stream);
diff --git a/xingtian_b200/capi.py b/xingtian_b200/capi.py
--- a/xingtian_b200/capi.py
+++ b/xingtian_b200/capi.py
@@ -165,6 +165,8 @@
     "xtb_comm_allreduce": (C.c_int, [_P, _P, C.c_longlong, _P]),
     "xtb_net_bench_layer": (C.c_int, [_P, C.c_int, C.c_int, _P, _P, C.c_int, _P]),
     "xtb_set_fuse_heads": (C.c_int, [C.c_int]),
+    "xtb_set_bwd_overlap": (C.c_int, [C.c_int]),
+    "xtb_set_gemm_cta_cap": (C.c_int, [C.c_int]),
     "xtb_set_tc_mode": (C.c_int, [C.c_int]),
     "xtb_get_tc_mode": (C.c_int, []),
     "xtb_tc_gemm_test": (C.c_int, [C.c_int, _P, _P, _P, C.c_int, C.c_int, C.c_int, C.c_int, _P]),
diff --git a/xingtian_b200/csrc/bp_gemm.cuh b/xingtian_b200/csrc/bp_gemm.cuh
--- a/xingtian_b200/csrc/bp_gemm.cuh
+++ b/xingtian_b200/csrc/bp_gemm.cuh
@@ -246,6 +246,7 @@
   int n_stage_ents;
   int kchunks, kc_split, n_ntiles;
   int n_units, n_btiles, B, N;
+  int n_vctas;
   BpT out; float* out_f32; int ld_f32; const float* bias; float alpha; int act;
   float* part; long long part_z; int ld_part;
   BpT src; int src_act; int accumulate; float* db_part;
@@ -285,6 +286,22 @@
   }
 };
 
+struct TileSeq {
+  int V, total, nbt, du, dbt, v, tile, u, bt;
+  __device__ __forceinline__ void init(int V_, int total_, int nbt_) {
+    V = V_; total = total_; nbt = nbt_; du = V / nbt; dbt = V - du * nbt;
+    v = (int)blockIdx.x; start();
+  }
+  __device__ __forceinline__ void start() { tile = v < V ? v : total; u = tile / nbt; bt = tile - u * nbt; }
+  __device__ __forceinline__ bool next() {
+    tile += V; u += du; bt += dbt;
+    if (bt >= nbt) { bt -= nbt; u++; }
+    if (tile < total) return false;
+    v += (int)gridDim.x; start();
+    return true;
+  }
+};
+
 template <int KIND, int N>
 __global__ void __launch_bounds__(RW_THREADS, 1)
 bp_rows_kernel(const __grid_constant__ RowsArgs a, int n_stages, int stage_bytes, int wres_bytes, int epi_banks) {
@@ -330,7 +347,6 @@
   const int total = a.n_units * a.n_btiles;
   constexpr bool CAT = (KIND != 2);
   const int nbt = a.n_btiles;
-  const int du = (int)gridDim.x / nbt, dbt = (int)gridDim.x - du * nbt;
 
   if (warp == BP_P_WARP) {
     const bool a_split = a.a_split != 0, w_res = a.w_res != 0;
@@ -341,7 +357,6 @@
     const char* w_lo = reinterpret_cast<const char*>(a.w_lo);
     constexpr int n_bh_fwd = N >> 3;
     int stage = 0; uint32_t phase = 0;
-    int u = (int)blockIdx.x / nbt, bt = (int)blockIdx.x - u * nbt;
     const int Bsz = a.B;
     TileWalk tw; tw.setup(a, stages_sm, units_sm);
     const int src_act = a.src_act, accumulate = a.accumulate;
@@ -351,8 +366,9 @@
     const char* o_lo = o_hi + a.out.lo_off * 2;
     const uint32_t s_ps = (uint32_t)a.src.pitch * 16u, o_ps = (uint32_t)a.out.pitch * 16u;
     int ebank = 0; uint32_t ephase = 0;
-    for (int tile = blockIdx.x; tile < total; tile += gridDim.x) {
-      const int b0 = bt * 128, nr = min(128, Bsz - b0);
+    TileSeq ts; ts.init(a.n_vctas, total, nbt);
+    for (; ts.tile < total; ts.next()) {
+      const int u = ts.u, b0 = ts.bt * 128, nr = min(128, Bsz - b0);
       const uint32_t a_bytes = (uint32_t)nr * 16u, row_off = (uint32_t)b0 * 16u;
       tw.init<KIND>(u);
       for (int s = 0; s < tw.ns; s++) {
@@ -407,8 +423,6 @@
         __syncwarp();
         if (++ebank == epi_banks) { ebank = 0; ephase ^= 1; }
       }
-      u += du; bt += dbt;
-      if (bt >= nbt) { bt -= nbt; u++; }
     }
   } else if (warp < BP_P_WARP) {
     constexpr int ACC = CAT ? 2 * N : N;
@@ -484,16 +498,34 @@
       if (++stage == n_stages) { stage = 0; phase ^= 1; }
     };
 
-    int tile = blockIdx.x;
-    int u = (int)blockIdx.x / nbt, bt = (int)blockIdx.x - u * nbt;
+    TileSeq ts; ts.init(a.n_vctas, total, nbt);
     TileWalk tw; tw.setup(a, stages_sm, units_sm);
     auto start_tile = [&](float* acc) {
-      tw.init<KIND>(u);
+      tw.init<KIND>(ts.u);
       tw.ns = __shfl_sync(0xffffffffu, tw.ns, 0);
       if (tw.ns == 0) return false;
       discard_regs<ACC / 2>(acc);
-      mma_stage(acc, tw.get(0), true, idle(bt));
+      mma_stage(acc, tw.get(0), true, idle(ts.bt));
       return true;
+    };
+    auto flush_db = [&](int v) {
+      asm volatile("bar.sync 1, %0;" ::"n"(32 * BP_CONSUMER_WARPS) : "memory");
+#pragma unroll
+      for (int j = 0; j < N / 4; j++) {
+        float s = dbacc[j];
+        s += __shfl_xor_sync(0xffffffffu, s, 4);
+        s += __shfl_xor_sync(0xffffffffu, s, 8);
+        s += __shfl_xor_sync(0xffffffffu, s, 16);
+        if (lane < 4) red_sh[warp][8 * (j >> 1) + 2 * lane + (j & 1)] = s;
+        dbacc[j] = 0.f;
+      }
+      asm volatile("bar.sync 1, %0;" ::"n"(32 * BP_CONSUMER_WARPS) : "memory");
+      if (tid < N) {
+        float t = 0.f;
+#pragma unroll
+        for (int w = 0; w < BP_CONSUMER_WARPS; w++) t += red_sh[w][tid];
+        a.db_part[(long long)v * N + tid] = t;
+      }
     };
 
     auto epilogue = [&](const float* cur, int cu, int cbt, bool empty, uint32_t eb) {
@@ -571,12 +603,11 @@
 
     constexpr bool OVERLAP = !(KIND == 0 && N == 64);
     auto finish_tile = [&](float* cur, float* nxt) {
-      for (int s = 1; s < tw.ns; s++) mma_stage(cur, tw.get(s), false, idle(bt));
+      for (int s = 1; s < tw.ns; s++) mma_stage(cur, tw.get(s), false, idle(ts.bt));
       const bool empty = tw.ns == 0;
-      const int cu = u, cbt = bt;
-      tile += gridDim.x; u += du; bt += dbt;
-      if (bt >= nbt) { bt -= nbt; u++; }
-      if (!(OVERLAP && tile < total && start_tile(nxt))) {
+      const int cu = ts.u, cbt = ts.bt, cv = ts.v;
+      const bool vend = ts.next();
+      if (!(OVERLAP && ts.tile < total && start_tile(nxt))) {
         wgmma_wait<0>();
         if (held >= 0 && lane == 0) mbar_arrive(empty0 + 8 * held);
         held = -1;
@@ -589,31 +620,15 @@
         if (lane == 0) mbar_arrive(eempty0 + 8 * ebank);
         if (++ebank == epi_banks) { ebank = 0; ephase ^= 1; }
       }
-      if (!OVERLAP && tile < total) start_tile(nxt);
+      if (KIND == 2 && a.db_part && vend) flush_db(cv);
+      if (!OVERLAP && ts.tile < total) start_tile(nxt);
     };
     float acc0[ACC / 2], acc1[ACC / 2];
-    if (tile < total) start_tile(acc0);
-    while (tile < total) {
+    if (ts.tile < total) start_tile(acc0);
+    while (ts.tile < total) {
       finish_tile(acc0, acc1);
-      if (tile >= total) break;
+      if (ts.tile >= total) break;
       finish_tile(acc1, acc0);
-    }
-    if (KIND == 2 && a.db_part) {
-#pragma unroll
-      for (int j = 0; j < N / 4; j++) {
-        float s = dbacc[j];
-        s += __shfl_xor_sync(0xffffffffu, s, 4);
-        s += __shfl_xor_sync(0xffffffffu, s, 8);
-        s += __shfl_xor_sync(0xffffffffu, s, 16);
-        if (lane < 4) red_sh[warp][8 * (j >> 1) + 2 * lane + (j & 1)] = s;
-      }
-      asm volatile("bar.sync 1, %0;" ::"n"(32 * BP_CONSUMER_WARPS) : "memory");
-      if (tid < N) {
-        float t = 0.f;
-#pragma unroll
-        for (int w = 0; w < BP_CONSUMER_WARPS; w++) t += red_sh[w][tid];
-        a.db_part[(long long)blockIdx.x * N + tid] = t;
-      }
     }
   }
 }
@@ -636,7 +651,7 @@
   BpT x; int x_split; BpT g; const bf16* zeros;
   int mode;
   const WgEnt* tab;
-  int R;
+  int R, S;
   int N, B, n_bsub, n_opix;
   int x_chunks, r_tiles, n_ntiles;
   float* part;
@@ -677,12 +692,15 @@
   pdl_wait();
   pdl_trigger();
   const uint32_t stage0 = smem_u32(smem);
-  const int n_slices = conv ? (int)gridDim.x / a.R : 1;
-  const int r_conv = conv ? (int)blockIdx.x / n_slices : 0, slice = conv ? (int)blockIdx.x - r_conv * n_slices : 0;
-  const int n_tiles = conv ? 1 : a.r_tiles * a.n_ntiles;
+  const int n_jobs = conv ? a.R * a.S : a.r_tiles * a.n_ntiles;
   const int n_kc = conv ? a.n_opix * a.n_bsub : a.n_bsub;
-  const int tile0 = conv ? 0 : (int)blockIdx.x, tile_step = conv ? 1 : (int)gridDim.x;
-  const int kc0 = conv ? slice : 0, kc_step = conv ? n_slices : 1;
+  const int kc_step = conv ? a.S : 1;
+  struct Job { int r, nt, kc0; };
+  auto job_of = [&](int j) {
+    if (conv) { const int r = j / a.S; return Job{r, 0, j - r * a.S}; }
+    const int rt = j / a.n_ntiles;
+    return Job{rt, j - rt * a.n_ntiles, 0};
+  };
 
   if (warp == BP_P_WARP) {
     const uint32_t pstride_x = (uint32_t)a.x.pitch * 16u, pstride_g = (uint32_t)a.g.pitch * 16u;
@@ -694,11 +712,12 @@
     const bool x_split = a.x_split != 0;
     constexpr int n_bh = N >> 3;
     int stage = 0; uint32_t phase = 0;
-    for (int tile = tile0; tile < n_tiles; tile += tile_step) {
-      const int rt = tile / a.n_ntiles, nt = tile - rt * a.n_ntiles;
-      for (int kc = kc0; kc < n_kc; kc += kc_step) {
+    for (int job = blockIdx.x; job < n_jobs; job += gridDim.x) {
+      const Job jb = job_of(job);
+      const int nt = jb.nt;
+      for (int kc = jb.kc0; kc < n_kc; kc += kc_step) {
         const int opix = conv ? kc / a.n_bsub : 0, bs = conv ? kc - opix * a.n_bsub : kc;
-        const WgEnt e = WgWalk::get(a, tab_sm, opix, r_conv, rt);
+        const WgEnt e = WgWalk::get(a, tab_sm, opix, jb.r, jb.r);
         if (!e.valid) continue;
         const int b0 = bs * WG_KB;
         const uint32_t bytes = (uint32_t)((min(WG_KB, a.B - b0) + 15) & ~15) * 16u, row_off = (uint32_t)b0 * 16u;
@@ -734,14 +753,15 @@
     const uint64_t desc = make_desc(0, 128, WG_PLANE);
     const uint32_t x_row_add = (uint32_t)(wg * 8 * WG_PLANE) >> 4;
     int stage = 0; uint32_t phase = 0;
-    for (int tile = tile0; tile < n_tiles; tile += tile_step) {
-      const int rt = tile / a.n_ntiles, nt = tile - rt * a.n_ntiles;
+    for (int job = blockIdx.x; job < n_jobs; job += gridDim.x) {
+      const Job jb = job_of(job);
+      const int rt = jb.r, nt = jb.nt;
 #pragma unroll
       for (int j = 0; j < N / 2; j++) acc[j] = 0.f;
       int held = -1;
-      for (int kc = kc0; kc < n_kc; kc += kc_step) {
+      for (int kc = jb.kc0; kc < n_kc; kc += kc_step) {
         const int opix = conv ? kc / a.n_bsub : 0, bs = conv ? kc - opix * a.n_bsub : kc;
-        if (!__shfl_sync(0xffffffffu, (int)WgWalk::get(a, tab_sm, opix, r_conv, rt).valid, 0)) continue;
+        if (!__shfl_sync(0xffffffffu, (int)WgWalk::get(a, tab_sm, opix, rt, rt).valid, 0)) continue;
         const int ksteps = __shfl_sync(0xffffffffu, ((min(WG_KB, a.B - bs * WG_KB) + 15) & ~15) >> 4, 0);
         mbar_wait(full0 + 8 * stage, phase);
         const uint32_t sA = stage0 + (uint32_t)stage * WG_STAGE;
@@ -778,7 +798,7 @@
         float* dst;
         bool ok;
         if (conv) {
-          dst = a.part + (((long long)slice * a.R + r_conv) * 128 + m) * N;
+          dst = a.part + (((long long)jb.kc0 * a.R + rt) * 128 + m) * N;
           ok = true;
         } else {
           const int k = rt * 128 + m;
diff --git a/xingtian_b200/csrc/xtb_engine.cu b/xingtian_b200/csrc/xtb_engine.cu
--- a/xingtian_b200/csrc/xtb_engine.cu
+++ b/xingtian_b200/csrc/xtb_engine.cu
@@ -711,6 +711,10 @@
   return e;
 }
 
+static int g_gemm_cap = 0;
+extern "C" int xtb_set_gemm_cta_cap(int cap) { g_gemm_cap = cap > 0 ? cap : 0; return XTB_OK; }
+static int gemm_grid(int work) { return std::max(1, g_gemm_cap > 0 ? std::min(work, g_gemm_cap) : std::min(work, kSMs)); }
+
 template <int KIND>
 static cudaError_t launch_rows(bp::RowsArgs& a, cudaStream_t st) {
   const auto kern = by_width(kRowsKernels<KIND>, a.N);
@@ -722,18 +726,19 @@
   if (m.n_stages < 2) return cudaErrorInvalidConfiguration;
   const int smem = 128 + m.wres_bytes + m.n_stages * m.stage_bytes + m.epi_banks * m.epi_bank_bytes + m.tab_bytes;
   const int total = a.n_units * a.n_btiles;
-  const int grid = std::min(total, kSMs);
-  XLAUNCH(kern, grid, bp::RW_THREADS, smem, st, a, m.n_stages, m.stage_bytes, m.wres_bytes, m.epi_banks);
+  a.n_vctas = std::min(total, kSMs);
+  XLAUNCH(kern, gemm_grid(a.n_vctas), bp::RW_THREADS, smem, st, a, m.n_stages, m.stage_bytes, m.wres_bytes, m.epi_banks);
   return cudaPeekAtLastError();
 }
 
-static cudaError_t launch_wgrad(const bp::WgradArgs& a, int grid, cudaStream_t st) {
+static int wgrad_jobs(const bp::WgradArgs& a) { return a.mode == 0 ? a.R * a.S : a.r_tiles * a.n_ntiles; }
+static cudaError_t launch_wgrad(const bp::WgradArgs& a, cudaStream_t st) {
   const auto kern = by_width(kWgradKernels, a.N);
   if (!kern) return cudaErrorInvalidValue;
   { cudaError_t e0 = ensure_kernel_attrs(); if (e0 != cudaSuccess) return e0; }
   const size_t smem = wgrad_smem(a.mode, a.n_opix, a.R);
   if (smem > (size_t)kMaxDynSmem) return cudaErrorInvalidConfiguration;
-  XLAUNCH(kern, grid, bp::WG_THREADS, (int)smem, st, a);
+  XLAUNCH(kern, gemm_grid(wgrad_jobs(a)), bp::WG_THREADS, (int)smem, st, a);
   return cudaPeekAtLastError();
 }
 
@@ -818,6 +823,9 @@
   return launch_rows<2>(a, st);
 }
 
+static int wgrad_slices(const LayerPlan& lp, int B) {
+  return std::max(1, std::min(kSMs / lp.R, lp.q.OH * lp.q.OW * ((B + bp::WG_KB - 1) / bp::WG_KB)));
+}
 static cudaError_t tc_wgrad(xtb_net* net, int i, int B, cudaStream_t st) {
   LayerPlan& lp = net->L[i];
   const int t = i + 1;
@@ -834,15 +842,51 @@
     a.tab = (const bp::WgEnt*)(net->ws + lp.wg_off);
     a.R = lp.R; a.N = lp.N; a.n_opix = q.OH * q.OW; a.n_ntiles = 1;
     a.part = (float*)(net->ws + lp.part_off);
-    const int slices = std::max(1, std::min(kSMs / lp.R, a.n_opix * a.n_bsub));
-    queue_reduction(net, a.part, slices, (long long)lp.R * 128 * lp.N, lp.R * 128 * lp.N, lp.w_off, nullptr, &lp);
-    return launch_wgrad(a, lp.R * slices, st);
+    a.S = wgrad_slices(lp, B);
+    queue_reduction(net, a.part, a.S, (long long)lp.R * 128 * lp.N, lp.R * 128 * lp.N, lp.w_off, nullptr, &lp);
+    return launch_wgrad(a, st);
   }
   a.mode = 1;
   a.N = std::min(lp.n_fwd, 64);
   a.x_chunks = lp.K / 8; a.r_tiles = (lp.K + 127) / 128; a.n_ntiles = lp.N / a.N; a.n_opix = 1; a.R = 1;
   a.dw = net->grads + lp.w_off; a.ldw = lp.N; a.k_rows = lp.K;
-  return launch_wgrad(a, std::min(kSMs, a.r_tiles * a.n_ntiles), st);
+  return launch_wgrad(a, st);
+}
+
+static int g_bwd_overlap = [] { const char* e = getenv("XTB_BWD_OVERLAP"); return e ? atoi(e) : 1; }();
+extern "C" int xtb_set_bwd_overlap(int mode) { g_bwd_overlap = mode; return XTB_OK; }
+
+static const int kOverlapMaxStagesPerSM = 32;
+static bool pair_overlaps(const LayerPlan& lp, int B) {
+  if (!g_bwd_overlap || !use_tc(lp) || lp.d.src == 0 || lp.d.kind == XTB_DUELING || lp.d.kind == XTB_LOGSTD) return false;
+  const int nbt = (B + 127) / 128, n_bsub = (B + bp::WG_KB - 1) / bp::WG_KB;
+  long long d_stages, w_stages;
+  if (lp.d.kind == XTB_CONV) {
+    d_stages = (long long)lp.dg_st.size() * nbt;
+    long long valid = 0;
+    for (const bp::WgEnt& e : lp.wg_tab) valid += e.valid;
+    w_stages = valid * n_bsub;
+  } else {
+    d_stages = (long long)(lp.K / lp.n_dg) * nbt * ((lp.N / 8 + 7) / 8);
+    w_stages = (long long)((lp.K + 127) / 128) * (lp.N / std::min(lp.n_fwd, 64)) * n_bsub;
+  }
+  return std::min(d_stages, w_stages) <= (long long)kSMs * kOverlapMaxStagesPerSM;
+}
+
+struct SideStream { cudaStream_t st = nullptr; cudaEvent_t fork = nullptr, join = nullptr; };
+static SideStream g_side_streams[64];
+static int side_stream(SideStream** out) {
+  int dev = 0;
+  CUDA_TRY(cudaGetDevice(&dev));
+  if (dev < 0 || dev >= 64) return fail(XTB_ERR_ARG, "device index %d out of range", dev);
+  SideStream& s = g_side_streams[dev];
+  if (!s.st) {
+    CUDA_TRY(cudaStreamCreateWithFlags(&s.st, cudaStreamNonBlocking));
+    CUDA_TRY(cudaEventCreateWithFlags(&s.fork, cudaEventDisableTiming));
+    CUDA_TRY(cudaEventCreateWithFlags(&s.join, cudaEventDisableTiming));
+  }
+  *out = &s;
+  return XTB_OK;
 }
 
 extern "C" int xtb_net_sync_weights(xtb_net* net, void* stream) {
@@ -953,7 +997,7 @@
     w.mode = 1; w.N = nt; w.B = K; w.n_bsub = (K + bp::WG_KB - 1) / bp::WG_KB; w.n_opix = 1; w.R = 1;
     w.x_chunks = M / 8; w.r_tiles = (M + 127) / 128; w.n_ntiles = N / nt;
     w.dw = c; w.ldw = N; w.k_rows = M;
-    e = launch_wgrad(w, std::min(kSMs, w.r_tiles * w.n_ntiles), st);
+    e = launch_wgrad(w, st);
   }
   g_launches.fetch_add(4, std::memory_order_relaxed);
   cudaError_t e2 = cudaStreamSynchronize(st);
@@ -1107,6 +1151,17 @@
   return XTB_OK;
 }
 
+static int wgrad_operands(xtb_net* net, int i, const void* obs, const int32_t* idx, int B, cudaStream_t st) {
+  const LayerPlan& lp = net->L[i];
+  const int t = i + 1;
+  if (use_tc(lp)) {
+    int rc = ensure_bp(net, t, B, true, st);
+    return rc ? rc : (lp.d.src == 0 ? op_decode(net, obs, idx, B, st) : ensure_bp(net, lp.d.src, B, false, st));
+  }
+  int rc = ensure_f32(net, t, B, true, st);
+  return rc || lp.d.src == 0 ? rc : ensure_f32(net, lp.d.src, B, false, st);
+}
+
 static int op_wgrad(xtb_net* net, int i, const void* obs, const int32_t* idx, int B, cudaStream_t st, bool bias_done = false) {
   const LayerPlan& lp = net->L[i];
   if (lp.d.kind == XTB_DUELING || lp.d.kind == XTB_LOGSTD) return XTB_OK;
@@ -1114,28 +1169,19 @@
   float* dw = net->grads + lp.w_off;
   float* db = net->grads + lp.b_off;
   const bool tc = use_tc(lp);
+  int rc = wgrad_operands(net, i, obs, idx, B, st);
+  if (rc) return rc;
   if (tc) {
-    int rc = ensure_bp(net, t, B, true, st);
-    if (rc) return rc;
-    rc = lp.d.src == 0 ? op_decode(net, obs, idx, B, st) : ensure_bp(net, lp.d.src, B, false, st);
-    if (rc) return rc;
     cudaError_t te = tc_wgrad(net, i, B, st);
     if (te != cudaSuccess) return fail(XTB_ERR_CUDA, "tensor-core wgrad launch (layer %d): %s", i, cudaGetErrorString(te));
   } else {
-    int rc = ensure_f32(net, t, B, true, st);
-    if (rc) return rc;
     const float* dy = gout_f32(net, t);
     auto gemm = [&](auto x, const int32_t* ix, float alpha) {
       if (lp.d.kind == XTB_CONV) conv_wgrad(lp, x, ix, dy, alpha, dw, B, st, !bias_done);
       else dense_wgrad(lp, x, ix, dy, alpha, dw, B, st, !bias_done);
     };
-    if (lp.d.src == 0) {
-      with_obs_type(net, obs, [&](auto x) { gemm(x, idx, net->desc.scale); });
-    } else {
-      rc = ensure_f32(net, lp.d.src, B, false, st);
-      if (rc) return rc;
-      gemm((const float*)out_f32(net, lp.d.src), nullptr, 1.f);
-    }
+    if (lp.d.src == 0) with_obs_type(net, obs, [&](auto x) { gemm(x, idx, net->desc.scale); });
+    else gemm((const float*)out_f32(net, lp.d.src), nullptr, 1.f);
   }
   LAUNCH_CHECK();
   if (bias_done || (!tc && (lp.d.src != 0 || net->desc.scale == 1.f))) return XTB_OK;
@@ -1318,6 +1364,8 @@
     if (!use_tc(c)) continue;
     if (ps.d.kind == XTB_CONV ? c.n_dg == ps.N : (c.d.kind == XTB_DENSE && c.n_dg == ps.N && c.K == ps.N)) fuse_bias[s] = 1;
   }
+  SideStream* side = nullptr;
+  bool forked = false;
   for (int i = nl - 1; i >= 0; i--) {
     if (o.skip & (1u << i)) continue;
     const LayerPlan& lp = net->L[i];
@@ -1325,11 +1373,20 @@
     if (!has_grad[t]) continue;
     const bool act_bwd = dy[t] && act_is_ext(lp.d.act);
     if (act_bwd) { int rc = act_backward(net, t, batch, st); if (rc) return rc; }
-    int rc = op_wgrad(net, i, obs, gather_idx, batch, st, fuse_bias[t] != 0 || act_bwd);
+    cudaStream_t wst = st;
+    if (pair_overlaps(lp, batch)) {
+      int rc = side ? XTB_OK : side_stream(&side);
+      if (!rc) rc = wgrad_operands(net, i, obs, gather_idx, batch, st);
+      if (rc) return rc;
+      CUDA_TRY(cudaEventRecord(side->fork, st));
+      CUDA_TRY(cudaStreamWaitEvent(side->st, side->fork, 0));
+      wst = side->st; forked = true;
+    }
+    int rc = op_wgrad(net, i, obs, gather_idx, batch, wst, fuse_bias[t] != 0 || act_bwd);
     if (rc) return rc;
     if (comm && comm->world > 1 && early_cnt == 0 && lp.d.kind == XTB_DENSE && use_tc(lp) && (long long)lp.K * lp.N >= (1 << 16)) {
       early_off = lp.w_off; early_cnt = (long long)lp.K * lp.N;
-      rc = comm_fork_allreduce(comm, net->grads + early_off, early_cnt, st);
+      rc = comm_fork_allreduce(comm, net->grads + early_off, early_cnt, wst);
       if (rc) return rc;
     }
     if (lp.d.kind == XTB_DUELING) {
@@ -1343,6 +1400,10 @@
       if (rc) return rc;
       written[s] = 1; has_grad[s] = 1; dy[s] = 1;
     }
+  }
+  if (forked) {
+    CUDA_TRY(cudaEventRecord(side->join, side->st));
+    CUDA_TRY(cudaStreamWaitEvent(st, side->join, 0));
   }
   if (o.dobs) {
     bool first = true;
@@ -1731,7 +1792,7 @@
 struct CaptureKey {
   uint64_t tag;
   const void* own[6];
-  uint64_t mode[2];
+  uint64_t mode[4];
   uint64_t arg[21];
   bool operator<(const CaptureKey& o) const { return memcmp(this, &o, sizeof(CaptureKey)) < 0; }
 };
@@ -1769,10 +1830,13 @@
 template <class F>
 static int run_graph(CaptureKey key, int use_graph, void* stream, F&& launch) {
   if (!use_graph) return launch(stream);
-  key.own[5] = g_comm; key.mode[0] = g_tc_mode; key.mode[1] = g_fuse_heads;
+  key.own[5] = g_comm; key.mode[0] = g_tc_mode; key.mode[1] = g_fuse_heads; key.mode[2] = g_bwd_overlap;
+  key.mode[3] = g_gemm_cap;
   StreamScope sc;
   int src = sc.begin(stream, true);
   if (src) return src;
+  SideStream* side = nullptr;
+  if (g_bwd_overlap) { src = side_stream(&side); if (src) return src; }
   auto it = g_graphs.find(key);
   if (it == g_graphs.end()) {
     cudaStream_t st = sc.st;
```

After: 292,100, median of 6. About the same (+1.2%).
